# argumentcomputer/lurk-beta

Hardware: AMD Instinct MI355X
Metric: MSM Mscalar-mul/s (Pallas Pedersen commitment, bases+scalars resident in HBM) (higher is better)
Workload: dtype u32x8 (255-bit Montgomery, integer VALU)

## Files before the change

### bench_tools/check_asm_operands.py

```python
#!/usr/bin/env python3
import re
import sys
import os
_CSRC = os.path.join(os.path.dirname(os.path.dirname(os.path.abspath(__file__))), 'lurk_beta_amd', 'csrc')
hdrs = [os.path.join(_CSRC, 'field29_mul_asm.cuh'), os.path.join(_CSRC, 'field_mul_asm.cuh')]
templates = []
for h in hdrs:
    src = open(h).read()
    for m in re.finditer(r'asm(?:\s+volatile)?\(\s*((?:\s*"[^"\n]*"\s*\n?)+)\s*:\s*([^;]*?);', src, re.S):
        lines = [l for l in re.findall(r'"([^"\n]*)"', m.group(1))]
        lines = [l.replace('\\n\\t', '').replace('\\n', '').strip() for l in lines]
        lines = [l for l in lines if l]
        cl = re.findall(r'"([vs]\d+)"', m.group(2).split(':')[-1])
        templates.append((lines, set(cl)))
print("templates:", [(len(t[0]), len(t[1])) for t in templates])
s = open(sys.argv[1]).read()
blocks = re.findall(r';;#ASMSTART\n(.*?);;#ASMEND', s, re.S)
print("asm blocks in .s:", len(blocks))
bad = 0
matched = 0
for b in blocks:
    bl = [l.strip() for l in b.strip().split('\n') if l.strip()]
    cand = [t for t in templates if len(t[0]) == len(bl)]
    if not cand:
        continue
    tl, clob = cand[0]
    for tl, clob in cand:
        ok = True
        ops = {}
        for a, e in zip(tl, bl):
            pat = re.escape(a)
            pat = re.sub(r'%(\d+)', lambda m: r'(?P<o' + m.group(1) + r'>\S+?)', pat.replace('\\%', '%'))
            seen = set()
            def fix(m):
                n = m.group(1)
                if n in seen: return '(?P=o%s)' % n
                seen.add(n); return m.group(0)
            pat = re.sub(r'\(\?P<o(\d+)>\\S\+\?\)', fix, pat)
            mm = re.fullmatch(pat, e)
            if not mm: ok = False; break
            ops.update(mm.groupdict())
        if ok:
            break
    if not ok:
        continue
    matched += 1
    clobnums = {(c[0], int(c[1:])) for c in clob}
    for k, r in ops.items():
        r = r.rstrip(',')
        m1 = re.fullmatch(r'([vs])(\d+)', r); m2 = re.fullmatch(r'([vs])\[(\d+):(\d+)\]', r)
        regs = []
        if m1: regs = [(m1.group(1), int(m1.group(2)))]
        elif m2: regs = [(m2.group(1), i) for i in range(int(m2.group(2)), int(m2.group(3)) + 1)]
        if any(x in clobnums for x in regs):
            bad += 1
            print("OVERLAP: operand %s -> %s is a clobbered scratch register" % (k, r))
print("matched blocks:", matched, "overlaps:", bad)
sys.exit(1 if bad or not matched else 0)
```

### lurk_beta_amd/csrc/curve29.cuh

```cuda
#pragma once
#include "curve.cuh"
#include "field29.cuh"

#ifndef LURK_ACC_Y3_ROW
#define LURK_ACC_Y3_ROW 1
#endif
#ifndef LURK_ACC_AFFINE_FIRST
#define LURK_ACC_AFFINE_FIRST 1
#endif
#ifndef LURK_F29_RARE_ATTR
#define LURK_F29_RARE_ATTR __attribute__((noinline))
#endif

namespace lurk {

template <class P>
LURK_HD F29<P> f29_carry_signed(const int32_t* t) {
    F29<P> r;
    int32_t c = 0;
#pragma unroll
    for (int i = 0; i < 8; i++) {
        int32_t x = t[i] + c;
        r.l[i] = (uint32_t)x & F29_MASK;
        c = x >> 29;
    }
    r.l[8] = (uint32_t)(t[8] + c);
    return r;
}

template <class P>
LURK_HD constexpr bool f29_pasta_shape() {
    return P::NBITS == 255 && f29_mod<P>(0) == 1u && f29_mod<P>(5) == 0u && f29_mod<P>(6) == 0u && f29_mod<P>(7) == 0u;
}

template <class P>
LURK_HD F29<P> f29_reduce_pasta(const F29<P>& v) {
    const uint32_t k = v.l[8] >> 22;
    const uint32_t km1 = k ? k - 1 : 0;
    int32_t t[9];
    uint64_t c = 0;
#pragma unroll
    for (int i = 0; i < 5; i++) {
        c += (uint64_t)km1 * f29_mod<P>(i);
        t[i] = (int32_t)v.l[i] - (int32_t)((uint32_t)c & F29_MASK);
        c >>= 29;
    }
    t[5] = (int32_t)v.l[5] - (int32_t)(uint32_t)c;
    t[6] = (int32_t)v.l[6];
    t[7] = (int32_t)v.l[7];
    t[8] = (int32_t)(v.l[8] & ((1u << 22) - 1u)) + (k ? (int32_t)(1u << 22) : 0);
    return f29_carry_signed<P>(t);
}
template <class P>
LURK_HD F29<P> f29_reduce_general(const F29<P>& v) {
    constexpr uint32_t D = (P::mod(7) >> 8) + 1u;
    static_assert(D > (1u << 21) && D <= (1u << 22), "f29_reduce_general: the modulus must have 253 or 254 bits");
    constexpr uint64_t mu = ((uint64_t)1 << 53) / D;
    F29_ASSERT(v.l[8] < (1u << 31), "f29_reduce: top limb >= 2^31");
    const uint32_t q = (uint32_t)(((uint64_t)v.l[8] * mu) >> 53);
    int32_t t[9];
    uint64_t c = 0;
#pragma unroll
    for (int i = 0; i < 8; i++) {
        c += (uint64_t)q * f29_mod<P>(i);
        t[i] = (int32_t)v.l[i] - (int32_t)((uint32_t)c & F29_MASK);
        c >>= 29;
    }
    c += (uint64_t)q * f29_mod<P>(8);
    t[8] = (int32_t)v.l[8] - (int32_t)(uint32_t)c;
    const F29<P> r = f29_carry_signed<P>(t);
    F29_ASSERT(r.l[8] < (1u << 24), "f29_reduce: result not below 2^256");
    return r;
}
template <class P>
LURK_HD F29<P> f29_reduce(const F29<P>& v) {
    if constexpr (f29_pasta_shape<P>()) return f29_reduce_pasta<P>(v);
    else return f29_reduce_general<P>(v);
}

template <class P>
struct Xyzz29 {
    F29<P> x, y, zz, zzz;
};

template <class P>
LURK_HD Xyzz<P> xyzz29_to_xyzz(const Xyzz29<P>& a, bool is_identity) {
    if (is_identity) return xyzz_identity<P>();
    Xyzz<P> r;
    r.x = f29_to_mont256<P>(a.x);
    r.y = f29_to_mont256<P>(a.y);
    r.zz = f29_to_mont256<P>(a.zz);
    r.zzz = f29_to_mont256<P>(a.zzz);
    return r;
}
template <class P>
LURK_HD void xyzz29_from_xyzz(const Xyzz<P>& a, Xyzz29<P>& r, bool& is_identity) {
    is_identity = xyzz_is_identity<P>(a);
    r.x = f29_from_mont256<P>(a.x);
    r.y = f29_from_mont256<P>(a.y);
    r.zz = f29_from_mont256<P>(a.zz);
    r.zzz = f29_from_mont256<P>(a.zzz);
}

template <class P>
LURK_HD uint32_t f29_multiple_candidate(const F29<P>& v) {
    if constexpr (f29_pasta_shape<P>()) return v.l[0];
    else return (v.l[0] * ((0u - f29_inv<P>()) & F29_MASK)) & F29_MASK;
}
template <class P>
LURK_HD bool f29_maybe_multiple_of_p(const F29<P>& v) {
    return f29_multiple_candidate<P>(v) < (f29_pasta_shape<P>() ? 128u : 256u);
}
template <class P>
LURK_HD bool f29_is_multiple_of_p(const F29<P>& v) {
    const uint32_t k = f29_multiple_candidate<P>(v);
    uint64_t c = 0;
    bool eq = true;
#pragma unroll
    for (int i = 0; i < 8; i++) {
        c += (uint64_t)k * f29_mod<P>(i);
        eq = eq && (v.l[i] == ((uint32_t)c & F29_MASK));
        c >>= 29;
    }
    c += (uint64_t)k * f29_mod<P>(8);
    return eq && (uint64_t)v.l[8] == c;
}

template <class P>
LURK_HD LURK_F29_RARE_ATTR Xyzz29<P> xyzz29_double_affine(F29<P> qx, F29<P> qy_signed) {
    const F29<P> u = f29_dbl<P>(qy_signed);
    const F29<P> v = f29_mul<P>(u, u);
    const F29<P> w = f29_mul<P>(u, v);
    const F29<P> s = f29_mul<P>(qx, v);
    const F29<P> xx = f29_sqr<P>(qx);
    const F29<P> m = f29_carry<P>(f29_add<P>(f29_dbl<P>(xx), xx));
    const F29<P> m2 = f29_sqr<P>(m);
    Xyzz29<P> r;
    r.x = f29_reduce<P>(f29_carry<P>(f29_sub<P>(m2, f29_dbl<P>(s))));
    const F29<P> t1 = f29_mul<P>(m, f29_sub<P>(s, r.x));
    const F29<P> t2 = f29_mul<P>(w, qy_signed);
    r.y = f29_reduce<P>(f29_carry<P>(f29_sub<P>(t1, t2)));
    r.zz = v;
    r.zzz = w;
    return r;
}

template <class P, bool ACC_AFFINE = false>
LURK_HD void xyzz29_madd(Xyzz29<P>& acc, bool& acc_id, const Affine<P>& q, bool negate) {
    if (affine_is_identity<P>(q)) return;
    const F29<P> qx = f29_from_mont256<P>(q.x);
    const F29<P> qy = f29_from_mont256<P>(q.y);
    if (acc_id) {
        acc.x = qx;
        acc.y = negate ? f29_reduce<P>(f29_carry<P>(f29_sub<P>(f29_zero<P>(), qy))) : qy;
        Fe<P> one = fe_one<P>();
        acc.zz = f29_from_mont256<P>(one);
        acc.zzz = acc.zz;
        acc_id = false;
        return;
    }
    F29_ASSERT_LIMBS(acc.x, 29, "acc.x"); F29_ASSERT_TOP(acc.x, 27, "acc.x");
    F29_ASSERT_LIMBS(acc.y, 29, "acc.y"); F29_ASSERT_TOP(acc.y, 27, "acc.y");
    F29_ASSERT_LIMBS(acc.zz, 29, "acc.zz"); F29_ASSERT_TOP(acc.zz, 27, "acc.zz");
    F29_ASSERT_LIMBS(acc.zzz, 29, "acc.zzz"); F29_ASSERT_TOP(acc.zzz, 27, "acc.zzz");
    const F29<P> u2 = ACC_AFFINE ? qx : f29_mul<P>(qx, acc.zz);
    const F29<P> s2 = ACC_AFFINE ? qy : f29_mul<P>(qy, acc.zzz);
    const F29<P> p = f29_carry<P>(f29_sub<P>(u2, acc.x));
    F29<P> r;
#pragma unroll
    for (int i = 0; i < 9; i++) {
        F29_ASSERT(f29_bias<P>(i) >= acc.y.l[i], "madd: Y1 limb above the bias");
        r.l[i] = s2.l[i] + (negate ? acc.y.l[i] : f29_bias<P>(i) - acc.y.l[i]);
    }
    r = f29_carry<P>(r);
    if (f29_maybe_multiple_of_p<P>(p) && f29_is_multiple_of_p<P>(p)) {
        if (f29_maybe_multiple_of_p<P>(r) && f29_is_multiple_of_p<P>(r)) {
            const F29<P> qys = negate ? f29_reduce<P>(f29_carry<P>(f29_sub<P>(f29_zero<P>(), qy))) : qy;
            acc = xyzz29_double_affine<P>(qx, qys);
        } else {
            acc_id = true;
        }
        return;
    }
    const F29<P> pp = f29_sqr<P>(p);
    const F29<P> ppp = f29_mul<P>(p, pp);
    const F29<P> qq = f29_mul<P>(acc.x, pp);
    const F29<P> r2 = f29_sqr<P>(r);
    F29<P> x3 = f29_sub<P>(f29_sub<P>(r2, ppp), f29_dbl<P>(qq));
    x3 = f29_reduce<P>(f29_carry<P>(x3));
    F29<P> d;
#pragma unroll
    for (int i = 0; i < 9; i++) {
        F29_ASSERT(f29_bias<P>(i) >= qq.l[i] && f29_bias<P>(i) >= x3.l[i], "madd: Q / X3 limb above the bias");
        d.l[i] = negate ? x3.l[i] + (f29_bias<P>(i) - qq.l[i]) : qq.l[i] + (f29_bias<P>(i) - x3.l[i]);
    }
#if LURK_ACC_Y3_ROW
    Dot29<P> row;
    dot29_init<P>(row);
    dot29_mac<P>(row, r, f29_carry<P>(d));
    dot29_mac<P>(row, f29_carry<P>(f29_sub<P>(f29_zero<P>(), acc.y)), ppp);
    F29<P> y3 = f29_reduce<P>(dot29_finish<P>(row));
#else
    const F29<P> t1 = f29_mul<P>(r, d);
    const F29<P> t2 = f29_mul<P>(acc.y, ppp);
    F29<P> y3 = f29_reduce<P>(f29_carry<P>(f29_sub<P>(t1, t2)));
#endif
    acc.x = x3;
    acc.y = y3;
    if (ACC_AFFINE) {
        acc.zz = f29_reduce<P>(pp);
        acc.zzz = f29_reduce<P>(ppp);
    } else {
        acc.zz = f29_mul<P>(acc.zz, pp);
        acc.zzz = f29_mul<P>(acc.zzz, ppp);
    }
}

template <class P>
LURK_HD Xyzz29<P> xyzz29_dbl(const Xyzz29<P>& a) {
    const F29<P> u = f29_dbl<P>(a.y);
    const F29<P> v = f29_mul<P>(u, u);
    const F29<P> w = f29_mul<P>(u, v);
    const F29<P> s = f29_mul<P>(a.x, v);
    const F29<P> xx = f29_sqr<P>(a.x);
    const F29<P> m = f29_carry<P>(f29_add<P>(f29_dbl<P>(xx), xx));
    const F29<P> m2 = f29_sqr<P>(m);
    Xyzz29<P> r;
    r.x = f29_reduce<P>(f29_carry<P>(f29_sub<P>(m2, f29_dbl<P>(s))));
    const F29<P> t1 = f29_mul<P>(m, f29_sub<P>(s, r.x));
    const F29<P> t2 = f29_mul<P>(w, a.y);
    r.y = f29_reduce<P>(f29_carry<P>(f29_sub<P>(t1, t2)));
    r.zz = f29_mul<P>(v, a.zz);
    r.zzz = f29_mul<P>(w, a.zzz);
    return r;
}

template <class P>
LURK_HD LURK_F29_RARE_ATTR Xyzz29<P> xyzz29_double_general(Xyzz29<P> a) {
    const Xyzz<P> d = xyzz_dbl<P>(xyzz29_to_xyzz<P>(a, false));
    Xyzz29<P> r;
    bool id;
    xyzz29_from_xyzz<P>(d, r, id);
    return r;
}

template <class P>
LURK_HD void xyzz29_add(Xyzz29<P>& acc, bool& acc_id, const Xyzz29<P>& q, bool q_id) {
    if (q_id) return;
    if (acc_id) {
        acc = q;
        acc_id = false;
        return;
    }
    F29_ASSERT_LIMBS(acc.x, 29, "add acc.x"); F29_ASSERT_TOP(acc.x, 27, "add acc.x");
    F29_ASSERT_LIMBS(acc.y, 29, "add acc.y"); F29_ASSERT_TOP(acc.y, 27, "add acc.y");
    F29_ASSERT_LIMBS(acc.zz, 29, "add acc.zz"); F29_ASSERT_TOP(acc.zz, 27, "add acc.zz");
    F29_ASSERT_LIMBS(acc.zzz, 29, "add acc.zzz"); F29_ASSERT_TOP(acc.zzz, 27, "add acc.zzz");
    F29_ASSERT_LIMBS(q.x, 29, "add q.x"); F29_ASSERT_TOP(q.x, 27, "add q.x");
    F29_ASSERT_LIMBS(q.y, 29, "add q.y"); F29_ASSERT_TOP(q.y, 27, "add q.y");
    F29_ASSERT_LIMBS(q.zz, 29, "add q.zz"); F29_ASSERT_TOP(q.zz, 27, "add q.zz");
    F29_ASSERT_LIMBS(q.zzz, 29, "add q.zzz"); F29_ASSERT_TOP(q.zzz, 27, "add q.zzz");
    const F29<P> u1 = f29_mul<P>(acc.x, q.zz);
    const F29<P> u2 = f29_mul<P>(q.x, acc.zz);
    const F29<P> s1 = f29_mul<P>(acc.y, q.zzz);
    const F29<P> s2 = f29_mul<P>(q.y, acc.zzz);
    const F29<P> p = f29_carry<P>(f29_sub<P>(u2, u1));
    const F29<P> r = f29_carry<P>(f29_sub<P>(s2, s1));
    if (f29_maybe_multiple_of_p<P>(p) && f29_is_multiple_of_p<P>(p)) {
        if (f29_maybe_multiple_of_p<P>(r) && f29_is_multiple_of_p<P>(r)) acc = xyzz29_double_general<P>(acc);
        else acc_id = true;
        return;
    }
    const F29<P> pp = f29_sqr<P>(p);
    const F29<P> ppp = f29_mul<P>(p, pp);
    const F29<P> qq = f29_mul<P>(u1, pp);
    const F29<P> r2 = f29_sqr<P>(r);
    F29<P> x3 = f29_sub<P>(f29_sub<P>(r2, ppp), f29_dbl<P>(qq));
    x3 = f29_reduce<P>(f29_carry<P>(x3));
    F29<P> d;
#pragma unroll
    for (int i = 0; i < 9; i++) {
        F29_ASSERT(f29_bias<P>(i) >= x3.l[i], "add: X3 limb above the bias");
        d.l[i] = qq.l[i] + (f29_bias<P>(i) - x3.l[i]);
    }
    Dot29<P> row;
    dot29_init<P>(row);
    dot29_mac<P>(row, r, f29_carry<P>(d));
    dot29_mac<P>(row, f29_carry<P>(f29_sub<P>(f29_zero<P>(), s1)), ppp);
    const F29<P> y3 = f29_reduce<P>(dot29_finish<P>(row));
    const F29<P> zz12 = f29_mul<P>(acc.zz, q.zz);
    const F29<P> zzz12 = f29_mul<P>(acc.zzz, q.zzz);
    acc.x = x3;
    acc.y = y3;
    acc.zz = f29_mul<P>(zz12, pp);
    acc.zzz = f29_mul<P>(zzz12, ppp);
}

template <class P>
LURK_HD Xyzz<P> xyzz_sum_via29(const Xyzz<P>* pts, uint32_t nt) {
    if (nt == 0) return xyzz_identity<P>();
    if (nt == 1) return pts[0];
    Xyzz29<P> acc, q;
    bool acc_id, q_id;
    xyzz29_from_xyzz<P>(pts[0], acc, acc_id);
    for (uint32_t i = 1; i < nt; i++) {
        xyzz29_from_xyzz<P>(pts[i], q, q_id);
        xyzz29_add<P>(acc, acc_id, q, q_id);
    }
    return xyzz29_to_xyzz<P>(acc, acc_id);
}

template <class P>
LURK_HD void msm_task_accumulate29_raw(const uint32_t* sorted, uint32_t first, uint32_t last, const Affine<P>* table, Xyzz29<P>& acc, bool& acc_id) {
    acc.x = acc.y = acc.zz = acc.zzz = f29_zero<P>();
    acc_id = true;
#if LURK_ACC_AFFINE_FIRST
    uint32_t j = first;
    if (j < last) {
        const uint32_t e = sorted[j++];
        xyzz29_madd<P>(acc, acc_id, table[e & 0x7fffffffu], (e & 0x80000000u) != 0);
    }
    if (j < last) {
        const uint32_t e = sorted[j++];
        const Affine<P> q = table[e & 0x7fffffffu];
#if LURK_ACC_AFFINE_FIRST
        if (!acc_id) xyzz29_madd<P, true>(acc, acc_id, q, (e & 0x80000000u) != 0);
        else
#endif
            xyzz29_madd<P>(acc, acc_id, q, (e & 0x80000000u) != 0);
    }
    for (; j < last; j++) {
        const uint32_t e = sorted[j];
        const Affine<P> q = table[e & 0x7fffffffu];
        xyzz29_madd<P>(acc, acc_id, q, (e & 0x80000000u) != 0);
    }
#else
    for (uint32_t j = first; j < last; j++) {
        const uint32_t e = sorted[j];
#ifdef LURK_ACC_DEBUG_TABLE_MASK
        const Affine<P> q = table[e & LURK_ACC_DEBUG_TABLE_MASK];
#else
        const Affine<P> q = table[e & 0x7fffffffu];
#endif
        xyzz29_madd<P>(acc, acc_id, q, (e & 0x80000000u) != 0);
    }
#endif
}
template <class P>
LURK_HD Xyzz<P> msm_task_accumulate29(const uint32_t* sorted, uint32_t first, uint32_t last, const Affine<P>* table) {
    Xyzz29<P> acc;
    bool acc_id;
    msm_task_accumulate29_raw<P>(sorted, first, last, table, acc, acc_id);
    return xyzz29_to_xyzz<P>(acc, acc_id);
}

}
```

### lurk_beta_amd/csrc/field29.cuh

```cuda
#pragma once
#include "field.cuh"

#if defined(LURK_F29_CHECK) && !defined(__HIP_DEVICE_COMPILE__)
#include <cstdio>
#include <cstdlib>
#define F29_CHECKS_ACTIVE 1
#define F29_ASSERT_LIMBS(v, bits, what)                                                        \
    do {                                                                                       \
        for (int _i = 0; _i < 9; _i++)                                                         \
            if ((uint64_t)(v).l[_i] >> (bits)) { printf("F29 bound violated: %s limb %d = %u (>= 2^%d)\n", what, _i, (v).l[_i], bits); abort(); } \
    } while (0)
#define F29_ASSERT(cond, what)                                                                 \
    do {                                                                                       \
        if (!(cond)) { printf("F29 bound violated: %s\n", what); abort(); }                     \
    } while (0)
#define F29_ASSERT_TOP(v, bits, what)                                                          \
    do {                                                                                       \
        if ((uint64_t)(v).l[8] >> (bits)) { printf("F29 bound violated: %s top limb = %u (>= 2^%d)\n", what, (v).l[8], bits); abort(); } \
    } while (0)
#else
#define F29_ASSERT_LIMBS(v, bits, what) ((void)0)
#define F29_ASSERT_TOP(v, bits, what) ((void)0)
#define F29_ASSERT(cond, what) ((void)0)
#define F29_CHECKS_ACTIVE 0
#endif


namespace lurk {

template <class P>
struct F29 {
    uint32_t l[9];
};

constexpr uint32_t F29_MASK = (1u << 29) - 1u;

template <class P>
LURK_HD constexpr uint32_t f29_mod(int i) {
    const int bit = 29 * i, limb = bit >> 5, sh = bit & 31;
    uint64_t v = limb < 8 ? P::mod(limb) : 0u;
    if (limb + 1 < 8) v |= (uint64_t)P::mod(limb + 1) << 32;
    return (uint32_t)(v >> sh) & F29_MASK;
}
template <class P>
LURK_HD constexpr uint32_t f29_inv() {
    return P::INV & F29_MASK;
}

template <class P>
LURK_HD F29<P> f29_zero() {
    F29<P> z;
#pragma unroll
    for (int i = 0; i < 9; i++) z.l[i] = 0;
    return z;
}

template <class P>
LURK_HD F29<P> f29_carry(const F29<P>& a) {
    F29<P> r;
    uint32_t c = 0;
#pragma unroll
    for (int i = 0; i < 8; i++) {
        uint32_t x = a.l[i] + c;
        r.l[i] = x & F29_MASK;
        c = x >> 29;
    }
    r.l[8] = a.l[8] + c;
    return r;
}

template <class P>
LURK_HD F29<P> f29_add(const F29<P>& a, const F29<P>& b) {
    F29<P> r;
#pragma unroll
    for (int i = 0; i < 9; i++) r.l[i] = a.l[i] + b.l[i];
    return r;
}
template <class P>
LURK_HD constexpr uint32_t f29_bias(int i) {
    uint64_t carry = 0;
    uint32_t limb = 0;
    for (int k = 0; k <= i; k++) {
        uint64_t x = (uint64_t)f29_mod<P>(k) * 64u + carry;
        limb = (uint32_t)(x & F29_MASK);
        carry = x >> 29;
        if (k == 8) limb = (uint32_t)x;
    }
    uint32_t v = limb;
    if (i < 8) v += 1u << 30;
    if (i > 0) v -= 2u;
    return v;
}
template <class P>
LURK_HD F29<P> f29_sub(const F29<P>& a, const F29<P>& b) {
    F29<P> r;
#pragma unroll
    for (int i = 0; i < 9; i++) {
        F29_ASSERT(f29_bias<P>(i) >= b.l[i], "f29_sub: subtrahend limb above the bias (value >= 64p or limbs not tight)");
        r.l[i] = a.l[i] + (f29_bias<P>(i) - b.l[i]);
    }
    return r;
}
template <class P>
LURK_HD F29<P> f29_dbl(const F29<P>& a) {
    F29<P> r;
#pragma unroll
    for (int i = 0; i < 9; i++) r.l[i] = a.l[i] << 1;
    return r;
}

template <class P>
LURK_HD F29<P> f29_mul_portable(const F29<P>& a, const F29<P>& b) {
    uint32_t m[9];
    F29<P> t;
    uint64_t acc = 0;
#if defined(LURK_F29_CHECK) && !defined(__HIP_DEVICE_COMPILE__)
    {
        uint64_t ma = 0, mb = 0;
        for (int i = 0; i < 9; i++) { ma = a.l[i] > ma ? a.l[i] : ma; mb = b.l[i] > mb ? b.l[i] : mb; }
        F29_ASSERT((unsigned __int128)ma * mb * 9 + ((unsigned __int128)10 << 58) < ((unsigned __int128)1 << 64), "f29_mul column overflow");
    }
#endif
#pragma unroll
    for (int k = 0; k < 17; k++) {
#pragma unroll
        for (int i = (k > 8 ? k - 8 : 0); i <= (k < 8 ? k : 8); i++) acc += (uint64_t)a.l[i] * b.l[k - i];
#pragma unroll
        for (int i = (k > 8 ? k - 8 : 0); i <= (k - 1 < 8 ? k - 1 : 8); i++) acc += (uint64_t)m[i] * f29_mod<P>(k - i);
        if (k <= 8) {
            m[k] = ((uint32_t)acc * f29_inv<P>()) & F29_MASK;
            acc += (uint64_t)m[k] * f29_mod<P>(0);
        } else {
            t.l[k - 9] = (uint32_t)acc & F29_MASK;
        }
        acc >>= 29;
    }
    t.l[8] = (uint32_t)acc;
    return t;
}

}
#include "field29_mul_asm.cuh"
#include "field29_mul_asm_bn254fq.cuh"
namespace lurk {

template <class P>
LURK_HD F29<P> f29_mul(const F29<P>& a, const F29<P>& b) {
#if defined(__HIP_DEVICE_COMPILE__)
    return f29_mul_asm<P>(a, b);
#else
    return f29_mul_portable<P>(a, b);
#endif
}
template <class P>
LURK_HD F29<P> f29_sqr(const F29<P>& a) {
#if defined(__HIP_DEVICE_COMPILE__)
    return f29_sqr_asm<P>(a);
#else
    return f29_mul_portable<P>(a, a);
#endif
}

template <class P>
LURK_HD F29<P> f29_invert(const F29<P>& a) {
    uint32_t e[8];
    uint32_t borrow = 2;
    for (int i = 0; i < 8; i++) {
        const uint64_t x = (uint64_t)P::mod(i) - borrow;
        e[i] = (uint32_t)x;
        borrow = (uint32_t)(x >> 63);
    }
    int top = 255;
    while (top > 0 && !((e[top >> 5] >> (top & 31)) & 1u)) top--;
    F29<P> acc = a;
#if defined(__HIP_DEVICE_COMPILE__)
#pragma unroll 1
#endif
    for (int b = top - 1; b >= 0; b--) {
        acc = f29_sqr<P>(acc);
        if ((e[b >> 5] >> (b & 31)) & 1u) acc = f29_mul<P>(acc, a);
    }
    return acc;
}

template <class P>
struct Dot29 {
    uint64_t c[17];
#if defined(LURK_F29_CHECK) && !defined(__HIP_DEVICE_COMPILE__)
    unsigned __int128 shadow[17];
#endif
};
template <class P>
LURK_HD void dot29_init(Dot29<P>& A) {
#pragma unroll
    for (int k = 0; k < 17; k++) A.c[k] = 0;
#if defined(LURK_F29_CHECK) && !defined(__HIP_DEVICE_COMPILE__)
    for (int k = 0; k < 17; k++) A.shadow[k] = 0;
#endif
}
template <class P>
LURK_HD void dot29_mac(Dot29<P>& A, const F29<P>& a, const F29<P>& b) {
#pragma unroll
    for (int i = 0; i < 9; i++)
#pragma unroll
        for (int j = 0; j < 9; j++) A.c[i + j] += (uint64_t)a.l[i] * b.l[j];
#if defined(LURK_F29_CHECK) && !defined(__HIP_DEVICE_COMPILE__)
    for (int i = 0; i < 9; i++)
        for (int j = 0; j < 9; j++) A.shadow[i + j] += (unsigned __int128)a.l[i] * b.l[j];
    for (int k = 0; k < 17; k++) F29_ASSERT(A.shadow[k] + ((unsigned __int128)10 << 58) < ((unsigned __int128)1 << 64), "dot29 column overflow");
#endif
}
template <class P>
LURK_HD void dot29_carry(Dot29<P>& A) {
#pragma unroll
    for (int k = 0; k < 16; k++) {
        A.c[k + 1] += A.c[k] >> 29;
        A.c[k] &= F29_MASK;
    }
#if defined(LURK_F29_CHECK) && !defined(__HIP_DEVICE_COMPILE__)
    for (int k = 0; k < 17; k++) A.shadow[k] = A.c[k];
#endif
}
template <class P>
LURK_HD F29<P> dot29_finish(const Dot29<P>& A) {
    uint32_t m[9];
    F29<P> t;
    uint64_t acc = 0;
#pragma unroll
    for (int k = 0; k < 17; k++) {
        acc += A.c[k];
#pragma unroll
        for (int i = (k > 8 ? k - 8 : 0); i <= (k - 1 < 8 ? k - 1 : 8); i++) acc += (uint64_t)m[i] * f29_mod<P>(k - i);
        if (k <= 8) {
            m[k] = ((uint32_t)acc * f29_inv<P>()) & F29_MASK;
            acc += (uint64_t)m[k] * f29_mod<P>(0);
        } else {
            t.l[k - 9] = (uint32_t)acc & F29_MASK;
        }
        acc >>= 29;
    }
    t.l[8] = (uint32_t)acc;
    return t;
}

template <class P>
LURK_HD F29<P> f29_from_mont256(const Fe<P>& x) {
    F29<P> r;
#pragma unroll
    for (int i = 0; i < 9; i++) {
        const int bit = 29 * i - 5;
        uint64_t v;
        if (bit < 0) {
            v = (uint64_t)x.l[0] << 5;
        } else {
            const int limb = bit >> 5, sh = bit & 31;
            v = limb < 8 ? x.l[limb] : 0u;
            if (limb + 1 < 8) v |= (uint64_t)x.l[limb + 1] << 32;
            v >>= sh;
        }
        r.l[i] = (uint32_t)v & F29_MASK;
    }
    return r;
}
template <class P>
LURK_HD F29<P> f29_from_plain(const uint32_t* x) {
    F29<P> r;
#pragma unroll
    for (int i = 0; i < 9; i++) {
        const int bit = 29 * i, limb = bit >> 5, sh = bit & 31;
        uint64_t v = limb < 8 ? x[limb] : 0u;
        if (limb + 1 < 8) v |= (uint64_t)x[limb + 1] << 32;
        r.l[i] = (uint32_t)(v >> sh) & F29_MASK;
    }
    return r;
}
template <class P>
LURK_HD void f29_pack(const F29<P>& a, uint32_t* out) {
#pragma unroll
    for (int w = 0; w < 8; w++) {
        const int bit = 32 * w, i = bit / 29, sh = bit % 29;
        uint64_t v = (uint64_t)a.l[i] >> sh;
        if (i + 1 < 9) v |= (uint64_t)a.l[i + 1] << (29 - sh);
        if (i + 2 < 9) v |= (uint64_t)a.l[i + 2] << (58 - sh);
        out[w] = (uint32_t)v;
    }
}
template <class P>
LURK_HD F29<P> f29_const_r256() {
    uint32_t r[8];
#pragma unroll
    for (int i = 0; i < 8; i++) r[i] = P::r(i);
    return f29_from_plain<P>(r);
}
template <class P>
LURK_HD Fe<P> f29_to_mont256(const F29<P>& a) {
    F29<P> u = f29_mul<P>(f29_carry<P>(a), f29_const_r256<P>());
    uint32_t w[8];
    f29_pack<P>(u, w);
    fe_cond_sub2<P>(w);
    fe_cond_sub<P>(w);
    Fe<P> r;
#pragma unroll
    for (int i = 0; i < 8; i++) r.l[i] = w[i];
    return r;
}

}
```

### lurk_beta_amd/csrc/gen_field29_asm.py

```python
#!/usr/bin/env python3
import sys

FIELDS = {
    "PallasFp": 0x40000000000000000000000000000000224698FC094CF91B992D30ED00000001,
    "PallasFq": 0x40000000000000000000000000000000224698FC0994A8DD8C46EB2100000001,
    "Bn254Fr": 0x30644E72E131A029B85045B68181585D2833E84879B9709143E1F593F0000001,
}
BN254FQ_FIELDS = {
    "Bn254Fq": 0x30644E72E131A029B85045B68181585D97816A916871CA8D3C208C16D87CFD47,
}
W = 29
MASK = (1 << W) - 1
ACC_LO, ACC_HI = 16, 17
M_BASE = 18
P_SGPR_BASE = 4
INV_SGPR = 13
MASK_VGPR = 27
DUMMY = 16
P_VGPR_BASE = 28
MOD_IN_VGPR = False
LAST_VGPR = P_VGPR_BASE + 8 if MOD_IN_VGPR else MASK_VGPR


def limbs29(x):
    return [(x >> (W * i)) & MASK for i in range(9)]


def gen_mul(modulus, square=False):
    p = limbs29(modulus)
    inv = (-pow(modulus, -1, 1 << W)) % (1 << W)
    L = []
    T = lambda i: f"%{i}"
    A = lambda i: f"%{9 + i}"
    B = lambda i: f"%{18 + i}"
    M = lambda i: f"v{M_BASE + i}"

    def P(j):
        if p[j] == 1:
            return "1"
        return f"v{P_VGPR_BASE + j}" if MOD_IN_VGPR else f"s{P_SGPR_BASE + j}"

    for j in range(9):
        if p[j] not in (0, 1):
            if MOD_IN_VGPR:
                L.append(f"v_mov_b32 v{P_VGPR_BASE + j}, 0x{p[j]:08x}")
            else:
                L.append(f"s_mov_b32 s{P_SGPR_BASE + j}, 0x{p[j]:08x}")
    if inv != MASK:
        L.append(f"s_mov_b32 s{INV_SGPR}, 0x{inv:08x}")
    L.append(f"v_mov_b32 v{MASK_VGPR}, 0x{MASK:08x}")
    first = True
    for k in range(17):
        if square:
            prods = [(A(i), B(k - i)) for i in range(max(0, k - 8), min(k, 8) + 1) if i < k - i]
            if k % 2 == 0:
                prods.append((A(k // 2), A(k // 2)))
        else:
            prods = [(A(i), B(k - i)) for i in range(max(0, k - 8), min(k, 8) + 1)]
        prods += [(M(i), P(k - i)) for i in range(max(0, k - 8), min(k - 1, 8) + 1) if p[k - i] != 0]
        for x, y in prods:
            src2 = "0" if first else f"v[{ACC_LO}:{ACC_HI}]"
            L.append(f"v_mad_u64_u32 v[{ACC_LO}:{ACC_HI}], s[{DUMMY}:{DUMMY + 1}], {x}, {y}, {src2}")
            first = False
        if k <= 8:
            if inv == MASK:
                L.append(f"v_sub_u32 {M(k)}, 0, v{ACC_LO}")
            else:
                L.append(f"v_mul_lo_u32 {M(k)}, v{ACC_LO}, s{INV_SGPR}")
            L.append(f"v_and_b32 {M(k)}, v{MASK_VGPR}, {M(k)}")
            L.append(f"v_mad_u64_u32 v[{ACC_LO}:{ACC_HI}], s[{DUMMY}:{DUMMY + 1}], {M(k)}, {P(0)}, v[{ACC_LO}:{ACC_HI}]")
        else:
            L.append(f"v_and_b32 {T(k - 9)}, v{MASK_VGPR}, v{ACC_LO}")
        if k < 16:
            L.append(f"v_lshrrev_b64 v[{ACC_LO}:{ACC_HI}], {W}, v[{ACC_LO}:{ACC_HI}]")
    L.append(f"v_lshrrev_b64 v[{ACC_LO}:{ACC_HI}], {W}, v[{ACC_LO}:{ACC_HI}]")
    L.append(f"v_mov_b32 {T(8)}, v{ACC_LO}")
    return L, p, inv


def cxx_sqr(name, modulus):
    lines, p, inv = gen_mul(modulus, square=True)
    nmad = sum(1 for l in lines if l.startswith("v_mad"))
    body = "\n".join(f'        "{l}\\n\\t"' for l in lines)
    outs = ", ".join(f'"=&v"(t.l[{i}])' for i in range(9))
    ins = ", ".join([f'"v"(a.l[{i}])' for i in range(9)] + [f'"v"(d.l[{i}])' for i in range(9)])
    vclob = ", ".join(f'"v{r}"' for r in range(ACC_LO, LAST_VGPR + 1))
    sclob = ", ".join(f'"s{r}"' for r in range(P_SGPR_BASE, DUMMY + 2))
    return f"""// {name} squaring: {nmad} v_mad_u64_u32 (cross products once, against the doubled operand)
template <>
__device__ __forceinline__ F29<{name}> f29_sqr_asm<{name}>(const F29<{name}>& a) {{
    F29<{name}> t, d;
#pragma unroll
    for (int i = 0; i < 9; i++) d.l[i] = a.l[i] << 1;
    asm(
{body}
        : {outs}
        : {ins}
        : {vclob}, {sclob}, "vcc");
    return t;
}}
"""


def cxx(name, modulus):
    lines, p, inv = gen_mul(modulus)
    nmad = sum(1 for l in lines if l.startswith("v_mad"))
    nvalu = sum(1 for l in lines if l.startswith("v_"))
    body = "\n".join(f'        "{l}\\n\\t"' for l in lines)
    outs = ", ".join(f'"=&v"(t.l[{i}])' for i in range(9))
    ins = ", ".join([f'"v"(a.l[{i}])' for i in range(9)] + [f'"v"(b.l[{i}])' for i in range(9)])
    vclob = ", ".join(f'"v{r}"' for r in range(ACC_LO, LAST_VGPR + 1))
    sclob = ", ".join(f'"s{r}"' for r in range(P_SGPR_BASE, DUMMY + 2))
    return f"""// {name}: {nmad} v_mad_u64_u32, {nvalu} VALU instructions, no carry folds
template <>
__device__ __forceinline__ F29<{name}> f29_mul_asm<{name}>(const F29<{name}>& a, const F29<{name}>& b) {{
    F29<{name}> t;
    asm(
{body}
        : {outs}
        : {ins}
        : {vclob}, {sclob}, "vcc");
    return t;
}}
"""


def main():
    bn254fq = sys.argv[1:] == ["--bn254fq"]
    out = [
        "// field29_mul_asm_bn254fq.cuh - GENERATED by gen_field29_asm.py --bn254fq; do not edit." if bn254fq else
        "// field29_mul_asm.cuh - GENERATED by gen_field29_asm.py; do not edit.",
        "#pragma once",
        "#if defined(__HIP_DEVICE_COMPILE__)",
        "namespace lurk {",
    ]
    if not bn254fq:
        out += [
            "template <class P> __device__ __forceinline__ F29<P> f29_mul_asm(const F29<P>& a, const F29<P>& b);",
            "template <class P> __device__ __forceinline__ F29<P> f29_sqr_asm(const F29<P>& a);",
        ]
    out.append("")
    for name, mod in (BN254FQ_FIELDS if bn254fq else FIELDS).items():
        out.append(cxx(name, mod))
        out.append(cxx_sqr(name, mod))
    out += ["}  // namespace lurk", "#endif"]
    sys.stdout.write("\n".join(out) + "\n")


if __name__ == "__main__":
    main()
```

Measured before the change: 1020.

## Add p≡1 mod 2^29 Montgomery variant using signed carry for Pasta field muls

Adds a second Montgomery multiply/square path for Pasta fields, whose modulus is 1 mod 2^29. It derives the per-column quotient with a bitwise NOT of a biased accumulator instead of a negate, and carries with an arithmetic shift. Most multiplications in the XYZZ add, double and madd formulas, plus the Y3 dot-row finish, now call this path through new mul30/sqr30 wrappers. The aim is to shorten the VALU instruction chain per field multiply, at the cost of tighter column-overflow bounds that now depend on operand limb sizes.

Result: faster. 1058 (median of 6 runs) (+3.8%).

```diff
diff --git a/bench_tools/check_asm_operands.py b/bench_tools/check_asm_operands.py
--- a/bench_tools/check_asm_operands.py
+++ b/bench_tools/check_asm_operands.py
@@ -3,7 +3,7 @@
 import sys
 import os
 _CSRC = os.path.join(os.path.dirname(os.path.dirname(os.path.abspath(__file__))), 'lurk_beta_amd', 'csrc')
-hdrs = [os.path.join(_CSRC, 'field29_mul_asm.cuh'), os.path.join(_CSRC, 'field_mul_asm.cuh')]
+hdrs = [os.path.join(_CSRC, 'field29_mul_asm.cuh'), os.path.join(_CSRC, 'field29_mul_asm_p1.cuh'), os.path.join(_CSRC, 'field_mul_asm.cuh')]
 templates = []
 for h in hdrs:
     src = open(h).read()
diff --git a/lurk_beta_amd/csrc/curve29.cuh b/lurk_beta_amd/csrc/curve29.cuh
--- a/lurk_beta_amd/csrc/curve29.cuh
+++ b/lurk_beta_amd/csrc/curve29.cuh
@@ -28,10 +28,6 @@
     return r;
 }
 
-template <class P>
-LURK_HD constexpr bool f29_pasta_shape() {
-    return P::NBITS == 255 && f29_mod<P>(0) == 1u && f29_mod<P>(5) == 0u && f29_mod<P>(6) == 0u && f29_mod<P>(7) == 0u;
-}
 
 template <class P>
 LURK_HD F29<P> f29_reduce_pasta(const F29<P>& v) {
@@ -130,15 +126,15 @@
 LURK_HD LURK_F29_RARE_ATTR Xyzz29<P> xyzz29_double_affine(F29<P> qx, F29<P> qy_signed) {
     const F29<P> u = f29_dbl<P>(qy_signed);
     const F29<P> v = f29_mul<P>(u, u);
-    const F29<P> w = f29_mul<P>(u, v);
-    const F29<P> s = f29_mul<P>(qx, v);
-    const F29<P> xx = f29_sqr<P>(qx);
+    const F29<P> w = f29_mul30<P>(u, v);
+    const F29<P> s = f29_mul30<P>(qx, v);
+    const F29<P> xx = f29_sqr30<P>(qx);
     const F29<P> m = f29_carry<P>(f29_add<P>(f29_dbl<P>(xx), xx));
-    const F29<P> m2 = f29_sqr<P>(m);
+    const F29<P> m2 = f29_sqr30<P>(m);
     Xyzz29<P> r;
     r.x = f29_reduce<P>(f29_carry<P>(f29_sub<P>(m2, f29_dbl<P>(s))));
     const F29<P> t1 = f29_mul<P>(m, f29_sub<P>(s, r.x));
-    const F29<P> t2 = f29_mul<P>(w, qy_signed);
+    const F29<P> t2 = f29_mul30<P>(w, qy_signed);
     r.y = f29_reduce<P>(f29_carry<P>(f29_sub<P>(t1, t2)));
     r.zz = v;
     r.zzz = w;
@@ -163,8 +159,8 @@
     F29_ASSERT_LIMBS(acc.y, 29, "acc.y"); F29_ASSERT_TOP(acc.y, 27, "acc.y");
     F29_ASSERT_LIMBS(acc.zz, 29, "acc.zz"); F29_ASSERT_TOP(acc.zz, 27, "acc.zz");
     F29_ASSERT_LIMBS(acc.zzz, 29, "acc.zzz"); F29_ASSERT_TOP(acc.zzz, 27, "acc.zzz");
-    const F29<P> u2 = ACC_AFFINE ? qx : f29_mul<P>(qx, acc.zz);
-    const F29<P> s2 = ACC_AFFINE ? qy : f29_mul<P>(qy, acc.zzz);
+    const F29<P> u2 = ACC_AFFINE ? qx : f29_mul30<P>(qx, acc.zz);
+    const F29<P> s2 = ACC_AFFINE ? qy : f29_mul30<P>(qy, acc.zzz);
     const F29<P> p = f29_carry<P>(f29_sub<P>(u2, acc.x));
     F29<P> r;
 #pragma unroll
@@ -182,10 +178,10 @@
         }
         return;
     }
-    const F29<P> pp = f29_sqr<P>(p);
-    const F29<P> ppp = f29_mul<P>(p, pp);
-    const F29<P> qq = f29_mul<P>(acc.x, pp);
-    const F29<P> r2 = f29_sqr<P>(r);
+    const F29<P> pp = f29_sqr30<P>(p);
+    const F29<P> ppp = f29_mul30<P>(p, pp);
+    const F29<P> qq = f29_mul30<P>(acc.x, pp);
+    const F29<P> r2 = f29_sqr30<P>(r);
     F29<P> x3 = f29_sub<P>(f29_sub<P>(r2, ppp), f29_dbl<P>(qq));
     x3 = f29_reduce<P>(f29_carry<P>(x3));
     F29<P> d;
@@ -199,10 +195,10 @@
     dot29_init<P>(row);
     dot29_mac<P>(row, r, f29_carry<P>(d));
     dot29_mac<P>(row, f29_carry<P>(f29_sub<P>(f29_zero<P>(), acc.y)), ppp);
-    F29<P> y3 = f29_reduce<P>(dot29_finish<P>(row));
+    F29<P> y3 = f29_reduce<P>(dot29_finish2<P>(row));
 #else
     const F29<P> t1 = f29_mul<P>(r, d);
-    const F29<P> t2 = f29_mul<P>(acc.y, ppp);
+    const F29<P> t2 = f29_mul30<P>(acc.y, ppp);
     F29<P> y3 = f29_reduce<P>(f29_carry<P>(f29_sub<P>(t1, t2)));
 #endif
     acc.x = x3;
@@ -211,8 +207,8 @@
         acc.zz = f29_reduce<P>(pp);
         acc.zzz = f29_reduce<P>(ppp);
     } else {
-        acc.zz = f29_mul<P>(acc.zz, pp);
-        acc.zzz = f29_mul<P>(acc.zzz, ppp);
+        acc.zz = f29_mul30<P>(acc.zz, pp);
+        acc.zzz = f29_mul30<P>(acc.zzz, ppp);
     }
 }
 
@@ -220,18 +216,18 @@
 LURK_HD Xyzz29<P> xyzz29_dbl(const Xyzz29<P>& a) {
     const F29<P> u = f29_dbl<P>(a.y);
     const F29<P> v = f29_mul<P>(u, u);
-    const F29<P> w = f29_mul<P>(u, v);
-    const F29<P> s = f29_mul<P>(a.x, v);
-    const F29<P> xx = f29_sqr<P>(a.x);
+    const F29<P> w = f29_mul30<P>(u, v);
+    const F29<P> s = f29_mul30<P>(a.x, v);
+    const F29<P> xx = f29_sqr30<P>(a.x);
     const F29<P> m = f29_carry<P>(f29_add<P>(f29_dbl<P>(xx), xx));
-    const F29<P> m2 = f29_sqr<P>(m);
+    const F29<P> m2 = f29_sqr30<P>(m);
     Xyzz29<P> r;
     r.x = f29_reduce<P>(f29_carry<P>(f29_sub<P>(m2, f29_dbl<P>(s))));
     const F29<P> t1 = f29_mul<P>(m, f29_sub<P>(s, r.x));
-    const F29<P> t2 = f29_mul<P>(w, a.y);
+    const F29<P> t2 = f29_mul30<P>(w, a.y);
     r.y = f29_reduce<P>(f29_carry<P>(f29_sub<P>(t1, t2)));
-    r.zz = f29_mul<P>(v, a.zz);
-    r.zzz = f29_mul<P>(w, a.zzz);
+    r.zz = f29_mul30<P>(v, a.zz);
+    r.zzz = f29_mul30<P>(w, a.zzz);
     return r;
 }
 
@@ -260,10 +256,10 @@
     F29_ASSERT_LIMBS(q.y, 29, "add q.y"); F29_ASSERT_TOP(q.y, 27, "add q.y");
     F29_ASSERT_LIMBS(q.zz, 29, "add q.zz"); F29_ASSERT_TOP(q.zz, 27, "add q.zz");
     F29_ASSERT_LIMBS(q.zzz, 29, "add q.zzz"); F29_ASSERT_TOP(q.zzz, 27, "add q.zzz");
-    const F29<P> u1 = f29_mul<P>(acc.x, q.zz);
-    const F29<P> u2 = f29_mul<P>(q.x, acc.zz);
-    const F29<P> s1 = f29_mul<P>(acc.y, q.zzz);
-    const F29<P> s2 = f29_mul<P>(q.y, acc.zzz);
+    const F29<P> u1 = f29_mul30<P>(acc.x, q.zz);
+    const F29<P> u2 = f29_mul30<P>(q.x, acc.zz);
+    const F29<P> s1 = f29_mul30<P>(acc.y, q.zzz);
+    const F29<P> s2 = f29_mul30<P>(q.y, acc.zzz);
     const F29<P> p = f29_carry<P>(f29_sub<P>(u2, u1));
     const F29<P> r = f29_carry<P>(f29_sub<P>(s2, s1));
     if (f29_maybe_multiple_of_p<P>(p) && f29_is_multiple_of_p<P>(p)) {
@@ -271,10 +267,10 @@
         else acc_id = true;
         return;
     }
-    const F29<P> pp = f29_sqr<P>(p);
-    const F29<P> ppp = f29_mul<P>(p, pp);
-    const F29<P> qq = f29_mul<P>(u1, pp);
-    const F29<P> r2 = f29_sqr<P>(r);
+    const F29<P> pp = f29_sqr30<P>(p);
+    const F29<P> ppp = f29_mul30<P>(p, pp);
+    const F29<P> qq = f29_mul30<P>(u1, pp);
+    const F29<P> r2 = f29_sqr30<P>(r);
     F29<P> x3 = f29_sub<P>(f29_sub<P>(r2, ppp), f29_dbl<P>(qq));
     x3 = f29_reduce<P>(f29_carry<P>(x3));
     F29<P> d;
@@ -287,13 +283,13 @@
     dot29_init<P>(row);
     dot29_mac<P>(row, r, f29_carry<P>(d));
     dot29_mac<P>(row, f29_carry<P>(f29_sub<P>(f29_zero<P>(), s1)), ppp);
-    const F29<P> y3 = f29_reduce<P>(dot29_finish<P>(row));
-    const F29<P> zz12 = f29_mul<P>(acc.zz, q.zz);
-    const F29<P> zzz12 = f29_mul<P>(acc.zzz, q.zzz);
+    const F29<P> y3 = f29_reduce<P>(dot29_finish2<P>(row));
+    const F29<P> zz12 = f29_mul30<P>(acc.zz, q.zz);
+    const F29<P> zzz12 = f29_mul30<P>(acc.zzz, q.zzz);
     acc.x = x3;
     acc.y = y3;
-    acc.zz = f29_mul<P>(zz12, pp);
-    acc.zzz = f29_mul<P>(zzz12, ppp);
+    acc.zz = f29_mul30<P>(zz12, pp);
+    acc.zzz = f29_mul30<P>(zzz12, ppp);
 }
 
 template <class P>
diff --git a/lurk_beta_amd/csrc/field29.cuh b/lurk_beta_amd/csrc/field29.cuh
--- a/lurk_beta_amd/csrc/field29.cuh
+++ b/lurk_beta_amd/csrc/field29.cuh
@@ -1,5 +1,9 @@
 #pragma once
 #include "field.cuh"
+
+#ifndef LURK_F29_P1
+#define LURK_F29_P1 1
+#endif
 
 #if defined(LURK_F29_CHECK) && !defined(__HIP_DEVICE_COMPILE__)
 #include <cstdio>
@@ -48,6 +52,15 @@
 }
 
 template <class P>
+LURK_HD constexpr bool f29_pasta_shape() {
+    return P::NBITS == 255 && f29_mod<P>(0) == 1u && f29_mod<P>(5) == 0u && f29_mod<P>(6) == 0u && f29_mod<P>(7) == 0u;
+}
+template <class P>
+LURK_HD constexpr bool f29_p1_form() {
+    return LURK_F29_P1 != 0 && f29_pasta_shape<P>() && f29_inv<P>() == F29_MASK;
+}
+
+template <class P>
 LURK_HD F29<P> f29_zero() {
     F29<P> z;
 #pragma unroll
@@ -139,9 +152,46 @@
     return t;
 }
 
+template <class P>
+LURK_HD F29<P> f29_mul30_portable(const F29<P>& a, const F29<P>& b) {
+    if constexpr (!f29_p1_form<P>()) {
+        return f29_mul_portable<P>(a, b);
+    } else {
+        uint32_t m[9];
+        F29<P> t;
+        uint64_t acc = ~(uint64_t)0;
+#if defined(LURK_F29_CHECK) && !defined(__HIP_DEVICE_COMPILE__)
+        {
+            uint64_t ma = 0, mb = 0;
+            for (int i = 0; i < 9; i++) { ma = a.l[i] > ma ? a.l[i] : ma; mb = b.l[i] > mb ? b.l[i] : mb; }
+            F29_ASSERT((unsigned __int128)ma * mb * 9 + ((unsigned __int128)5 << 58) + ((unsigned __int128)1 << 36) < ((unsigned __int128)1 << 63), "f29_mul column overflow");
+        }
+#endif
+#pragma unroll
+        for (int k = 0; k < 17; k++) {
+#pragma unroll
+            for (int i = (k > 8 ? k - 8 : 0); i <= (k < 8 ? k : 8); i++) acc += (uint64_t)a.l[i] * b.l[k - i];
+#pragma unroll
+            for (int i = (k > 8 ? k - 8 : 0); i <= (k - 1 < 8 ? k - 1 : 8); i++) acc += (uint64_t)m[i] * f29_mod<P>(k - i);
+            if (k <= 8) {
+                F29_ASSERT((int64_t)acc >= -1, "f29_mul column overflow");
+                m[k] = ~(uint32_t)acc & F29_MASK;
+                acc = (uint64_t)((int64_t)acc >> 29);
+                if (k == 8) acc += 1;
+            } else {
+                t.l[k - 9] = (uint32_t)acc & F29_MASK;
+                acc >>= 29;
+            }
+        }
+        t.l[8] = (uint32_t)acc;
+        return t;
+    }
+}
+
 }
 #include "field29_mul_asm.cuh"
 #include "field29_mul_asm_bn254fq.cuh"
+#include "field29_mul_asm_p1.cuh"
 namespace lurk {
 
 template <class P>
@@ -153,11 +203,29 @@
 #endif
 }
 template <class P>
+LURK_HD F29<P> f29_mul30(const F29<P>& a, const F29<P>& b) {
+#if defined(__HIP_DEVICE_COMPILE__)
+    if constexpr (f29_p1_form<P>()) return f29_mul_p1_asm<P>(a, b);
+    else return f29_mul_asm<P>(a, b);
+#else
+    return f29_mul30_portable<P>(a, b);
+#endif
+}
+template <class P>
 LURK_HD F29<P> f29_sqr(const F29<P>& a) {
 #if defined(__HIP_DEVICE_COMPILE__)
     return f29_sqr_asm<P>(a);
 #else
     return f29_mul_portable<P>(a, a);
+#endif
+}
+template <class P>
+LURK_HD F29<P> f29_sqr30(const F29<P>& a) {
+#if defined(__HIP_DEVICE_COMPILE__)
+    if constexpr (f29_p1_form<P>()) return f29_sqr_p1_asm<P>(a);
+    else return f29_sqr_asm<P>(a);
+#else
+    return f29_mul30_portable<P>(a, a);
 #endif
 }
 
@@ -177,8 +245,8 @@
 #pragma unroll 1
 #endif
     for (int b = top - 1; b >= 0; b--) {
-        acc = f29_sqr<P>(acc);
-        if ((e[b >> 5] >> (b & 31)) & 1u) acc = f29_mul<P>(acc, a);
+        acc = f29_sqr30<P>(acc);
+        if ((e[b >> 5] >> (b & 31)) & 1u) acc = f29_mul30<P>(acc, a);
     }
     return acc;
 }
@@ -241,6 +309,38 @@
     }
     t.l[8] = (uint32_t)acc;
     return t;
+}
+
+template <class P>
+LURK_HD F29<P> dot29_finish2(const Dot29<P>& A) {
+    if constexpr (!f29_p1_form<P>()) {
+        return dot29_finish<P>(A);
+    } else {
+        uint32_t m[9];
+        F29<P> t;
+        uint64_t acc = ~(uint64_t)0;
+#if defined(LURK_F29_CHECK) && !defined(__HIP_DEVICE_COMPILE__)
+        for (int k = 0; k < 17; k++)
+            F29_ASSERT(A.shadow[k] + ((unsigned __int128)5 << 58) + ((unsigned __int128)1 << 36) < ((unsigned __int128)1 << 63), "dot29 column overflow");
+#endif
+#pragma unroll
+        for (int k = 0; k < 17; k++) {
+            acc += A.c[k];
+#pragma unroll
+            for (int i = (k > 8 ? k - 8 : 0); i <= (k - 1 < 8 ? k - 1 : 8); i++) acc += (uint64_t)m[i] * f29_mod<P>(k - i);
+            if (k <= 8) {
+                F29_ASSERT((int64_t)acc >= -1, "dot29 column overflow");
+                m[k] = ~(uint32_t)acc & F29_MASK;
+                acc = (uint64_t)((int64_t)acc >> 29);
+                if (k == 8) acc += 1;
+            } else {
+                t.l[k - 9] = (uint32_t)acc & F29_MASK;
+                acc >>= 29;
+            }
+        }
+        t.l[8] = (uint32_t)acc;
+        return t;
+    }
 }
 
 template <class P>
@@ -294,7 +394,7 @@
 }
 template <class P>
 LURK_HD Fe<P> f29_to_mont256(const F29<P>& a) {
-    F29<P> u = f29_mul<P>(f29_carry<P>(a), f29_const_r256<P>());
+    F29<P> u = f29_mul30<P>(f29_carry<P>(a), f29_const_r256<P>());
     uint32_t w[8];
     f29_pack<P>(u, w);
     fe_cond_sub2<P>(w);
diff --git a/lurk_beta_amd/csrc/field29_mul_asm_p1.cuh b/lurk_beta_amd/csrc/field29_mul_asm_p1.cuh
--- /dev/null
+++ b/lurk_beta_amd/csrc/field29_mul_asm_p1.cuh
@@ -0,0 +1,688 @@
+#pragma once
+#if defined(__HIP_DEVICE_COMPILE__)
+namespace lurk {
+template <class P> __device__ __forceinline__ F29<P> f29_mul_p1_asm(const F29<P>& a, const F29<P>& b);
+template <class P> __device__ __forceinline__ F29<P> f29_sqr_p1_asm(const F29<P>& a);
+
+template <>
+__device__ __forceinline__ F29<PallasFp> f29_mul_p1_asm<PallasFp>(const F29<PallasFp>& a, const F29<PallasFp>& b) {
+    F29<PallasFp> t;
+    asm(
+        "s_mov_b32 s5, 0x09698768\n\t"
+        "s_mov_b32 s6, 0x133e46e6\n\t"
+        "s_mov_b32 s7, 0x0d31f812\n\t"
+        "s_mov_b32 s8, 0x00000224\n\t"
+        "s_mov_b32 s12, 0x00400000\n\t"
+        "v_mov_b32 v27, 0x1fffffff\n\t"
+        "v_mad_u64_u32 v[16:17], s[16:17], %9, %18, -1\n\t"
+        "v_not_b32 v18, v16\n\t"
+        "v_and_b32 v18, v27, v18\n\t"
+        "v_ashrrev_i64 v[16:17], 29, v[16:17]\n\t"
+        "v_mad_u64_u32 v[16:17], s[16:17], %9, %19, v[16:17]\n\t"
+        "v_mad_u64_u32 v[16:17], s[16:17], %10, %18, v[16:17]\n\t"
+        "v_mad_u64_u32 v[16:17], s[16:17], v18, s5, v[16:17]\n\t"
+        "v_not_b32 v19, v16\n\t"
+        "v_and_b32 v19, v27, v19\n\t"
+        "v_ashrrev_i64 v[16:17], 29, v[16:17]\n\t"
+        "v_mad_u64_u32 v[16:17], s[16:17], %9, %20, v[16:17]\n\t"
+        "v_mad_u64_u32 v[16:17], s[16:17], %10, %19, v[16:17]\n\t"
+        "v_mad_u64_u32 v[16:17], s[16:17], %11, %18, v[16:17]\n\t"
+        "v_mad_u64_u32 v[16:17], s[16:17], v18, s6, v[16:17]\n\t"
+        "v_mad_u64_u32 v[16:17], s[16:17], v19, s5, v[16:17]\n\t"
+        "v_not_b32 v20, v16\n\t"
+        "v_and_b32 v20, v27, v20\n\t"
+        "v_ashrrev_i64 v[16:17], 29, v[16:17]\n\t"
+        "v_mad_u64_u32 v[16:17], s[16:17], %9, %21, v[16:17]\n\t"
+        "v_mad_u64_u32 v[16:17], s[16:17], %10, %20, v[16:17]\n\t"
+        "v_mad_u64_u32 v[16:17], s[16:17], %11, %19, v[16:17]\n\t"
+        "v_mad_u64_u32 v[16:17], s[16:17], %12, %18, v[16:17]\n\t"
+        "v_mad_u64_u32 v[16:17], s[16:17], v18, s7, v[16:17]\n\t"
+        "v_mad_u64_u32 v[16:17], s[16:17], v19, s6, v[16:17]\n\t"
+        "v_mad_u64_u32 v[16:17], s[16:17], v20, s5, v[16:17]\n\t"
+        "v_not_b32 v21, v16\n\t"
+        "v_and_b32 v21, v27, v21\n\t"
+        "v_ashrrev_i64 v[16:17], 29, v[16:17]\n\t"
+        "v_mad_u64_u32 v[16:17], s[16:17], %9, %22, v[16:17]\n\t"
+        "v_mad_u64_u32 v[16:17], s[16:17], %10, %21, v[16:17]\n\t"
+        "v_mad_u64_u32 v[16:17], s[16:17], %11, %20, v[16:17]\n\t"
+        "v_mad_u64_u32 v[16:17], s[16:17], %12, %19, v[16:17]\n\t"
+        "v_mad_u64_u32 v[16:17], s[16:17], %13, %18, v[16:17]\n\t"
+        "v_mad_u64_u32 v[16:17], s[16:17], v18, s8, v[16:17]\n\t"
+        "v_mad_u64_u32 v[16:17], s[16:17], v19, s7, v[16:17]\n\t"
+        "v_mad_u64_u32 v[16:17], s[16:17], v20, s6, v[16:17]\n\t"
+        "v_mad_u64_u32 v[16:17], s[16:17], v21, s5, v[16:17]\n\t"
+        "v_not_b32 v22, v16\n\t"
+        "v_and_b32 v22, v27, v22\n\t"
+        "v_ashrrev_i64 v[16:17], 29, v[16:17]\n\t"
+        "v_mad_u64_u32 v[16:17], s[16:17], %9, %23, v[16:17]\n\t"
+        "v_mad_u64_u32 v[16:17], s[16:17], %10, %22, v[16:17]\n\t"
+        "v_mad_u64_u32 v[16:17], s[16:17], %11, %21, v[16:17]\n\t"
+        "v_mad_u64_u32 v[16:17], s[16:17], %12, %20, v[16:17]\n\t"
+        "v_mad_u64_u32 v[16:17], s[16:17], %13, %19, v[16:17]\n\t"
+        "v_mad_u64_u32 v[16:17], s[16:17], %14, %18, v[16:17]\n\t"
+        "v_mad_u64_u32 v[16:17], s[16:17], v19, s8, v[16:17]\n\t"
+        "v_mad_u64_u32 v[16:17], s[16:17], v20, s7, v[16:17]\n\t"
+        "v_mad_u64_u32 v[16:17], s[16:17], v21, s6, v[16:17]\n\t"
+        "v_mad_u64_u32 v[16:17], s[16:17], v22, s5, v[16:17]\n\t"
+        "v_not_b32 v23, v16\n\t"
+        "v_and_b32 v23, v27, v23\n\t"
+        "v_ashrrev_i64 v[16:17], 29, v[16:17]\n\t"
+        "v_mad_u64_u32 v[16:17], s[16:17], %9, %24, v[16:17]\n\t"
+        "v_mad_u64_u32 v[16:17], s[16:17], %10, %23, v[16:17]\n\t"
+        "v_mad_u64_u32 v[16:17], s[16:17], %11, %22, v[16:17]\n\t"
+        "v_mad_u64_u32 v[16:17], s[16:17], %12, %21, v[16:17]\n\t"
+        "v_mad_u64_u32 v[16:17], s[16:17], %13, %20, v[16:17]\n\t"
+        "v_mad_u64_u32 v[16:17], s[16:17], %14, %19, v[16:17]\n\t"
+        "v_mad_u64_u32 v[16:17], s[16:17], %15, %18, v[16:17]\n\t"
+        "v_mad_u64_u32 v[16:17], s[16:17], v20, s8, v[16:17]\n\t"
+        "v_mad_u64_u32 v[16:17], s[16:17], v21, s7, v[16:17]\n\t"
+        "v_mad_u64_u32 v[16:17], s[16:17], v22, s6, v[16:17]\n\t"
+        "v_mad_u64_u32 v[16:17], s[16:17], v23, s5, v[16:17]\n\t"
+        "v_not_b32 v24, v16\n\t"
+        "v_and_b32 v24, v27, v24\n\t"
+        "v_ashrrev_i64 v[16:17], 29, v[16:17]\n\t"
+        "v_mad_u64_u32 v[16:17], s[16:17], %9, %25, v[16:17]\n\t"
+        "v_mad_u64_u32 v[16:17], s[16:17], %10, %24, v[16:17]\n\t"
+        "v_mad_u64_u32 v[16:17], s[16:17], %11, %23, v[16:17]\n\t"
+        "v_mad_u64_u32 v[16:17], s[16:17], %12, %22, v[16:17]\n\t"
+        "v_mad_u64_u32 v[16:17], s[16:17], %13, %21, v[16:17]\n\t"
+        "v_mad_u64_u32 v[16:17], s[16:17], %14, %20, v[16:17]\n\t"
+        "v_mad_u64_u32 v[16:17], s[16:17], %15, %19, v[16:17]\n\t"
+        "v_mad_u64_u32 v[16:17], s[16:17], %16, %18, v[16:17]\n\t"
+        "v_mad_u64_u32 v[16:17], s[16:17], v21, s8, v[16:17]\n\t"
+        "v_mad_u64_u32 v[16:17], s[16:17], v22, s7, v[16:17]\n\t"
+        "v_mad_u64_u32 v[16:17], s[16:17], v23, s6, v[16:17]\n\t"
+        "v_mad_u64_u32 v[16:17], s[16:17], v24, s5, v[16:17]\n\t"
+        "v_not_b32 v25, v16\n\t"
+        "v_and_b32 v25, v27, v25\n\t"
+        "v_ashrrev_i64 v[16:17], 29, v[16:17]\n\t"
+        "v_mad_u64_u32 v[16:17], s[16:17], %9, %26, v[16:17]\n\t"
+        "v_mad_u64_u32 v[16:17], s[16:17], %10, %25, v[16:17]\n\t"
+        "v_mad_u64_u32 v[16:17], s[16:17], %11, %24, v[16:17]\n\t"
+        "v_mad_u64_u32 v[16:17], s[16:17], %12, %23, v[16:17]\n\t"
+        "v_mad_u64_u32 v[16:17], s[16:17], %13, %22, v[16:17]\n\t"
+        "v_mad_u64_u32 v[16:17], s[16:17], %14, %21, v[16:17]\n\t"
+        "v_mad_u64_u32 v[16:17], s[16:17], %15, %20, v[16:17]\n\t"
+        "v_mad_u64_u32 v[16:17], s[16:17], %16, %19, v[16:17]\n\t"
+        "v_mad_u64_u32 v[16:17], s[16:17], %17, %18, v[16:17]\n\t"
+        "v_mad_u64_u32 v[16:17], s[16:17], v18, s12, v[16:17]\n\t"
+        "v_mad_u64_u32 v[16:17], s[16:17], v22, s8, v[16:17]\n\t"
+        "v_mad_u64_u32 v[16:17], s[16:17], v23, s7, v[16:17]\n\t"
+        "v_mad_u64_u32 v[16:17], s[16:17], v24, s6, v[16:17]\n\t"
+        "v_mad_u64_u32 v[16:17], s[16:17], v25, s5, v[16:17]\n\t"
+        "v_not_b32 v26, v16\n\t"
+        "v_and_b32 v26, v27, v26\n\t"
+        "v_ashrrev_i64 v[16:17], 29, v[16:17]\n\t"
+        "v_lshl_add_u64 v[16:17], v[16:17], 0, 1\n\t"
+        "v_mad_u64_u32 v[16:17], s[16:17], %10, %26, v[16:17]\n\t"
+        "v_mad_u64_u32 v[16:17], s[16:17], %11, %25, v[16:17]\n\t"
+        "v_mad_u64_u32 v[16:17], s[16:17], %12, %24, v[16:17]\n\t"
+        "v_mad_u64_u32 v[16:17], s[16:17], %13, %23, v[16:17]\n\t"
+        "v_mad_u64_u32 v[16:17], s[16:17], %14, %22, v[16:17]\n\t"
+        "v_mad_u64_u32 v[16:17], s[16:17], %15, %21, v[16:17]\n\t"
+        "v_mad_u64_u32 v[16:17], s[16:17], %16, %20, v[16:17]\n\t"
+        "v_mad_u64_u32 v[16:17], s[16:17], %17, %19, v[16:17]\n\t"
+        "v_mad_u64_u32 v[16:17], s[16:17], v19, s12, v[16:17]\n\t"
+        "v_mad_u64_u32 v[16:17], s[16:17], v23, s8, v[16:17]\n\t"
+        "v_mad_u64_u32 v[16:17], s[16:17], v24, s7, v[16:17]\n\t"
+        "v_mad_u64_u32 v[16:17], s[16:17], v25, s6, v[16:17]\n\t"
+        "v_mad_u64_u32 v[16:17], s[16:17], v26, s5, v[16:17]\n\t"
+        "v_and_b32 %0, v27, v16\n\t"
+        "v_lshrrev_b64 v[16:17], 29, v[16:17]\n\t"
+        "v_mad_u64_u32 v[16:17], s[16:17], %11, %26, v[16:17]\n\t"
+        "v_mad_u64_u32 v[16:17], s[16:17], %12, %25, v[16:17]\n\t"
+        "v_mad_u64_u32 v[16:17], s[16:17], %13, %24, v[16:17]\n\t"
+        "v_mad_u64_u32 v[16:17], s[16:17], %14, %23, v[16:17]\n\t"
+        "v_mad_u64_u32 v[16:17], s[16:17], %15, %22, v[16:17]\n\t"
+        "v_mad_u64_u32 v[16:17], s[16:17], %16, %21, v[16:17]\n\t"
+        "v_mad_u64_u32 v[16:17], s[16:17], %17, %20, v[16:17]\n\t"
+        "v_mad_u64_u32 v[16:17], s[16:17], v20, s12, v[16:17]\n\t"
+        "v_mad_u64_u32 v[16:17], s[16:17], v24, s8, v[16:17]\n\t"
+        "v_mad_u64_u32 v[16:17], s[16:17], v25, s7, v[16:17]\n\t"
+        "v_mad_u64_u32 v[16:17], s[16:17], v26, s6, v[16:17]\n\t"
+        "v_and_b32 %1, v27, v16\n\t"
+        "v_lshrrev_b64 v[16:17], 29, v[16:17]\n\t"
+        "v_mad_u64_u32 v[16:17], s[16:17], %12, %26, v[16:17]\n\t"
+        "v_mad_u64_u32 v[16:17], s[16:17], %13, %25, v[16:17]\n\t"
+        "v_mad_u64_u32 v[16:17], s[16:17], %14, %24, v[16:17]\n\t"
+        "v_mad_u64_u32 v[16:17], s[16:17], %15, %23, v[16:17]\n\t"
+        "v_mad_u64_u32 v[16:17], s[16:17], %16, %22, v[16:17]\n\t"
+        "v_mad_u64_u32 v[16:17], s[16:17], %17, %21, v[16:17]\n\t"
+        "v_mad_u64_u32 v[16:17], s[16:17], v21, s12, v[16:17]\n\t"
+        "v_mad_u64_u32 v[16:17], s[16:17], v25, s8, v[16:17]\n\t"
+        "v_mad_u64_u32 v[16:17], s[16:17], v26, s7, v[16:17]\n\t"
+        "v_and_b32 %2, v27, v16\n\t"
+        "v_lshrrev_b64 v[16:17], 29, v[16:17]\n\t"
+        "v_mad_u64_u32 v[16:17], s[16:17], %13, %26, v[16:17]\n\t"
+        "v_mad_u64_u32 v[16:17], s[16:17], %14, %25, v[16:17]\n\t"
+        "v_mad_u64_u32 v[16:17], s[16:17], %15, %24, v[16:17]\n\t"
+        "v_mad_u64_u32 v[16:17], s[16:17], %16, %23, v[16:17]\n\t"
+        "v_mad_u64_u32 v[16:17], s[16:17], %17, %22, v[16:17]\n\t"
+        "v_mad_u64_u32 v[16:17], s[16:17], v22, s12, v[16:17]\n\t"
+        "v_mad_u64_u32 v[16:17], s[16:17], v26, s8, v[16:17]\n\t"
+        "v_and_b32 %3, v27, v16\n\t"
+        "v_lshrrev_b64 v[16:17], 29, v[16:17]\n\t"
+        "v_mad_u64_u32 v[16:17], s[16:17], %14, %26, v[16:17]\n\t"
+        "v_mad_u64_u32 v[16:17], s[16:17], %15, %25, v[16:17]\n\t"
+        "v_mad_u64_u32 v[16:17], s[16:17], %16, %24, v[16:17]\n\t"
+        "v_mad_u64_u32 v[16:17], s[16:17], %17, %23, v[16:17]\n\t"
+        "v_mad_u64_u32 v[16:17], s[16:17], v23, s12, v[16:17]\n\t"
+        "v_and_b32 %4, v27, v16\n\t"
+        "v_lshrrev_b64 v[16:17], 29, v[16:17]\n\t"
+        "v_mad_u64_u32 v[16:17], s[16:17], %15, %26, v[16:17]\n\t"
+        "v_mad_u64_u32 v[16:17], s[16:17], %16, %25, v[16:17]\n\t"
+        "v_mad_u64_u32 v[16:17], s[16:17], %17, %24, v[16:17]\n\t"
+        "v_mad_u64_u32 v[16:17], s[16:17], v24, s12, v[16:17]\n\t"
+        "v_and_b32 %5, v27, v16\n\t"
+        "v_lshrrev_b64 v[16:17], 29, v[16:17]\n\t"
+        "v_mad_u64_u32 v[16:17], s[16:17], %16, %26, v[16:17]\n\t"
+        "v_mad_u64_u32 v[16:17], s[16:17], %17, %25, v[16:17]\n\t"
+        "v_mad_u64_u32 v[16:17], s[16:17], v25, s12, v[16:17]\n\t"
+        "v_and_b32 %6, v27, v16\n\t"
+        "v_lshrrev_b64 v[16:17], 29, v[16:17]\n\t"
+        "v_mad_u64_u32 v[16:17], s[16:17], %17, %26, v[16:17]\n\t"
+        "v_mad_u64_u32 v[16:17], s[16:17], v26, s12, v[16:17]\n\t"
+        "v_and_b32 %7, v27, v16\n\t"
+        "v_lshrrev_b64 v[16:17], 29, v[16:17]\n\t"
+        "v_mov_b32 %8, v16\n\t"
+        : "=&v"(t.l[0]), "=&v"(t.l[1]), "=&v"(t.l[2]), "=&v"(t.l[3]), "=&v"(t.l[4]), "=&v"(t.l[5]), "=&v"(t.l[6]), "=&v"(t.l[7]), "=&v"(t.l[8])
+        : "v"(a.l[0]), "v"(a.l[1]), "v"(a.l[2]), "v"(a.l[3]), "v"(a.l[4]), "v"(a.l[5]), "v"(a.l[6]), "v"(a.l[7]), "v"(a.l[8]), "v"(b.l[0]), "v"(b.l[1]), "v"(b.l[2]), "v"(b.l[3]), "v"(b.l[4]), "v"(b.l[5]), "v"(b.l[6]), "v"(b.l[7]), "v"(b.l[8])
+        : "v16", "v17", "v18", "v19", "v20", "v21", "v22", "v23", "v24", "v25", "v26", "v27", "s4", "s5", "s6", "s7", "s8", "s9", "s10", "s11", "s12", "s13", "s14", "s15", "s16", "s17", "vcc");
+    return t;
+}
+
+template <>
+__device__ __forceinline__ F29<PallasFp> f29_sqr_p1_asm<PallasFp>(const F29<PallasFp>& a) {
+    F29<PallasFp> t, d;
+#pragma unroll
+    for (int i = 0; i < 9; i++) d.l[i] = a.l[i] << 1;
+    asm(
+        "s_mov_b32 s5, 0x09698768\n\t"
+        "s_mov_b32 s6, 0x133e46e6\n\t"
+        "s_mov_b32 s7, 0x0d31f812\n\t"
+        "s_mov_b32 s8, 0x00000224\n\t"
+        "s_mov_b32 s12, 0x00400000\n\t"
+        "v_mov_b32 v27, 0x1fffffff\n\t"
+        "v_mad_u64_u32 v[16:17], s[16:17], %9, %9, -1\n\t"
+        "v_not_b32 v18, v16\n\t"
+        "v_and_b32 v18, v27, v18\n\t"
+        "v_ashrrev_i64 v[16:17], 29, v[16:17]\n\t"
+        "v_mad_u64_u32 v[16:17], s[16:17], %9, %19, v[16:17]\n\t"
+        "v_mad_u64_u32 v[16:17], s[16:17], v18, s5, v[16:17]\n\t"
+        "v_not_b32 v19, v16\n\t"
+        "v_and_b32 v19, v27, v19\n\t"
+        "v_ashrrev_i64 v[16:17], 29, v[16:17]\n\t"
+        "v_mad_u64_u32 v[16:17], s[16:17], %9, %20, v[16:17]\n\t"
+        "v_mad_u64_u32 v[16:17], s[16:17], %10, %10, v[16:17]\n\t"
+        "v_mad_u64_u32 v[16:17], s[16:17], v18, s6, v[16:17]\n\t"
+        "v_mad_u64_u32 v[16:17], s[16:17], v19, s5, v[16:17]\n\t"
+        "v_not_b32 v20, v16\n\t"
+        "v_and_b32 v20, v27, v20\n\t"
+        "v_ashrrev_i64 v[16:17], 29, v[16:17]\n\t"
+        "v_mad_u64_u32 v[16:17], s[16:17], %9, %21, v[16:17]\n\t"
+        "v_mad_u64_u32 v[16:17], s[16:17], %10, %20, v[16:17]\n\t"
+        "v_mad_u64_u32 v[16:17], s[16:17], v18, s7, v[16:17]\n\t"
+        "v_mad_u64_u32 v[16:17], s[16:17], v19, s6, v[16:17]\n\t"
+        "v_mad_u64_u32 v[16:17], s[16:17], v20, s5, v[16:17]\n\t"
+        "v_not_b32 v21, v16\n\t"
+        "v_and_b32 v21, v27, v21\n\t"
+        "v_ashrrev_i64 v[16:17], 29, v[16:17]\n\t"
+        "v_mad_u64_u32 v[16:17], s[16:17], %9, %22, v[16:17]\n\t"
+        "v_mad_u64_u32 v[16:17], s[16:17], %10, %21, v[16:17]\n\t"
+        "v_mad_u64_u32 v[16:17], s[16:17], %11, %11, v[16:17]\n\t"
+        "v_mad_u64_u32 v[16:17], s[16:17], v18, s8, v[16:17]\n\t"
+        "v_mad_u64_u32 v[16:17], s[16:17], v19, s7, v[16:17]\n\t"
+        "v_mad_u64_u32 v[16:17], s[16:17], v20, s6, v[16:17]\n\t"
+        "v_mad_u64_u32 v[16:17], s[16:17], v21, s5, v[16:17]\n\t"
+        "v_not_b32 v22, v16\n\t"
+        "v_and_b32 v22, v27, v22\n\t"
+        "v_ashrrev_i64 v[16:17], 29, v[16:17]\n\t"
+        "v_mad_u64_u32 v[16:17], s[16:17], %9, %23, v[16:17]\n\t"
+        "v_mad_u64_u32 v[16:17], s[16:17], %10, %22, v[16:17]\n\t"
+        "v_mad_u64_u32 v[16:17], s[16:17], %11, %21, v[16:17]\n\t"
+        "v_mad_u64_u32 v[16:17], s[16:17], v19, s8, v[16:17]\n\t"
+        "v_mad_u64_u32 v[16:17], s[16:17], v20, s7, v[16:17]\n\t"
+        "v_mad_u64_u32 v[16:17], s[16:17], v21, s6, v[16:17]\n\t"
+        "v_mad_u64_u32 v[16:17], s[16:17], v22, s5, v[16:17]\n\t"
+        "v_not_b32 v23, v16\n\t"
+        "v_and_b32 v23, v27, v23\n\t"
+        "v_ashrrev_i64 v[16:17], 29, v[16:17]\n\t"
+        "v_mad_u64_u32 v[16:17], s[16:17], %9, %24, v[16:17]\n\t"
+        "v_mad_u64_u32 v[16:17], s[16:17], %10, %23, v[16:17]\n\t"
+        "v_mad_u64_u32 v[16:17], s[16:17], %11, %22, v[16:17]\n\t"
+        "v_mad_u64_u32 v[16:17], s[16:17], %12, %12, v[16:17]\n\t"
+        "v_mad_u64_u32 v[16:17], s[16:17], v20, s8, v[16:17]\n\t"
+        "v_mad_u64_u32 v[16:17], s[16:17], v21, s7, v[16:17]\n\t"
+        "v_mad_u64_u32 v[16:17], s[16:17], v22, s6, v[16:17]\n\t"
+        "v_mad_u64_u32 v[16:17], s[16:17], v23, s5, v[16:17]\n\t"
+        "v_not_b32 v24, v16\n\t"
+        "v_and_b32 v24, v27, v24\n\t"
+        "v_ashrrev_i64 v[16:17], 29, v[16:17]\n\t"
+        "v_mad_u64_u32 v[16:17], s[16:17], %9, %25, v[16:17]\n\t"
+        "v_mad_u64_u32 v[16:17], s[16:17], %10, %24, v[16:17]\n\t"
+        "v_mad_u64_u32 v[16:17], s[16:17], %11, %23, v[16:17]\n\t"
+        "v_mad_u64_u32 v[16:17], s[16:17], %12, %22, v[16:17]\n\t"
+        "v_mad_u64_u32 v[16:17], s[16:17], v21, s8, v[16:17]\n\t"
+        "v_mad_u64_u32 v[16:17], s[16:17], v22, s7, v[16:17]\n\t"
+        "v_mad_u64_u32 v[16:17], s[16:17], v23, s6, v[16:17]\n\t"
+        "v_mad_u64_u32 v[16:17], s[16:17], v24, s5, v[16:17]\n\t"
+        "v_not_b32 v25, v16\n\t"
+        "v_and_b32 v25, v27, v25\n\t"
+        "v_ashrrev_i64 v[16:17], 29, v[16:17]\n\t"
+        "v_mad_u64_u32 v[16:17], s[16:17], %9, %26, v[16:17]\n\t"
+        "v_mad_u64_u32 v[16:17], s[16:17], %10, %25, v[16:17]\n\t"
+        "v_mad_u64_u32 v[16:17], s[16:17], %11, %24, v[16:17]\n\t"
+        "v_mad_u64_u32 v[16:17], s[16:17], %12, %23, v[16:17]\n\t"
+        "v_mad_u64_u32 v[16:17], s[16:17], %13, %13, v[16:17]\n\t"
+        "v_mad_u64_u32 v[16:17], s[16:17], v18, s12, v[16:17]\n\t"
+        "v_mad_u64_u32 v[16:17], s[16:17], v22, s8, v[16:17]\n\t"
+        "v_mad_u64_u32 v[16:17], s[16:17], v23, s7, v[16:17]\n\t"
+        "v_mad_u64_u32 v[16:17], s[16:17], v24, s6, v[16:17]\n\t"
+        "v_mad_u64_u32 v[16:17], s[16:17], v25, s5, v[16:17]\n\t"
+        "v_not_b32 v26, v16\n\t"
+        "v_and_b32 v26, v27, v26\n\t"
+        "v_ashrrev_i64 v[16:17], 29, v[16:17]\n\t"
+        "v_lshl_add_u64 v[16:17], v[16:17], 0, 1\n\t"
+        "v_mad_u64_u32 v[16:17], s[16:17], %10, %26, v[16:17]\n\t"
+        "v_mad_u64_u32 v[16:17], s[16:17], %11, %25, v[16:17]\n\t"
+        "v_mad_u64_u32 v[16:17], s[16:17], %12, %24, v[16:17]\n\t"
+        "v_mad_u64_u32 v[16:17], s[16:17], %13, %23, v[16:17]\n\t"
+        "v_mad_u64_u32 v[16:17], s[16:17], v19, s12, v[16:17]\n\t"
+        "v_mad_u64_u32 v[16:17], s[16:17], v23, s8, v[16:17]\n\t"
+        "v_mad_u64_u32 v[16:17], s[16:17], v24, s7, v[16:17]\n\t"
+        "v_mad_u64_u32 v[16:17], s[16:17], v25, s6, v[16:17]\n\t"
+        "v_mad_u64_u32 v[16:17], s[16:17], v26, s5, v[16:17]\n\t"
+        "v_and_b32 %0, v27, v16\n\t"
+        "v_lshrrev_b64 v[16:17], 29, v[16:17]\n\t"
+        "v_mad_u64_u32 v[16:17], s[16:17], %11, %26, v[16:17]\n\t"
+        "v_mad_u64_u32 v[16:17], s[16:17], %12, %25, v[16:17]\n\t"
+        "v_mad_u64_u32 v[16:17], s[16:17], %13, %24, v[16:17]\n\t"
+        "v_mad_u64_u32 v[16:17], s[16:17], %14, %14, v[16:17]\n\t"
+        "v_mad_u64_u32 v[16:17], s[16:17], v20, s12, v[16:17]\n\t"
+        "v_mad_u64_u32 v[16:17], s[16:17], v24, s8, v[16:17]\n\t"
+        "v_mad_u64_u32 v[16:17], s[16:17], v25, s7, v[16:17]\n\t"
+        "v_mad_u64_u32 v[16:17], s[16:17], v26, s6, v[16:17]\n\t"
+        "v_and_b32 %1, v27, v16\n\t"
+        "v_lshrrev_b64 v[16:17], 29, v[16:17]\n\t"
+        "v_mad_u64_u32 v[16:17], s[16:17], %12, %26, v[16:17]\n\t"
+        "v_mad_u64_u32 v[16:17], s[16:17], %13, %25, v[16:17]\n\t"
+        "v_mad_u64_u32 v[16:17], s[16:17], %14, %24, v[16:17]\n\t"
+        "v_mad_u64_u32 v[16:17], s[16:17], v21, s12, v[16:17]\n\t"
+        "v_mad_u64_u32 v[16:17], s[16:17], v25, s8, v[16:17]\n\t"
+        "v_mad_u64_u32 v[16:17], s[16:17], v26, s7, v[16:17]\n\t"
+        "v_and_b32 %2, v27, v16\n\t"
+        "v_lshrrev_b64 v[16:17], 29, v[16:17]\n\t"
+        "v_mad_u64_u32 v[16:17], s[16:17], %13, %26, v[16:17]\n\t"
+        "v_mad_u64_u32 v[16:17], s[16:17], %14, %25, v[16:17]\n\t"
+        "v_mad_u64_u32 v[16:17], s[16:17], %15, %15, v[16:17]\n\t"
+        "v_mad_u64_u32 v[16:17], s[16:17], v22, s12, v[16:17]\n\t"
+        "v_mad_u64_u32 v[16:17], s[16:17], v26, s8, v[16:17]\n\t"
+        "v_and_b32 %3, v27, v16\n\t"
+        "v_lshrrev_b64 v[16:17], 29, v[16:17]\n\t"
+        "v_mad_u64_u32 v[16:17], s[16:17], %14, %26, v[16:17]\n\t"
+        "v_mad_u64_u32 v[16:17], s[16:17], %15, %25, v[16:17]\n\t"
+        "v_mad_u64_u32 v[16:17], s[16:17], v23, s12, v[16:17]\n\t"
+        "v_and_b32 %4, v27, v16\n\t"
+        "v_lshrrev_b64 v[16:17], 29, v[16:17]\n\t"
+        "v_mad_u64_u32 v[16:17], s[16:17], %15, %26, v[16:17]\n\t"
+        "v_mad_u64_u32 v[16:17], s[16:17], %16, %16, v[16:17]\n\t"
+        "v_mad_u64_u32 v[16:17], s[16:17], v24, s12, v[16:17]\n\t"
+        "v_and_b32 %5, v27, v16\n\t"
+        "v_lshrrev_b64 v[16:17], 29, v[16:17]\n\t"
+        "v_mad_u64_u32 v[16:17], s[16:17], %16, %26, v[16:17]\n\t"
+        "v_mad_u64_u32 v[16:17], s[16:17], v25, s12, v[16:17]\n\t"
+        "v_and_b32 %6, v27, v16\n\t"
+        "v_lshrrev_b64 v[16:17], 29, v[16:17]\n\t"
+        "v_mad_u64_u32 v[16:17], s[16:17], %17, %17, v[16:17]\n\t"
+        "v_mad_u64_u32 v[16:17], s[16:17], v26, s12, v[16:17]\n\t"
+        "v_and_b32 %7, v27, v16\n\t"
+        "v_lshrrev_b64 v[16:17], 29, v[16:17]\n\t"
+        "v_mov_b32 %8, v16\n\t"
+        : "=&v"(t.l[0]), "=&v"(t.l[1]), "=&v"(t.l[2]), "=&v"(t.l[3]), "=&v"(t.l[4]), "=&v"(t.l[5]), "=&v"(t.l[6]), "=&v"(t.l[7]), "=&v"(t.l[8])
+        : "v"(a.l[0]), "v"(a.l[1]), "v"(a.l[2]), "v"(a.l[3]), "v"(a.l[4]), "v"(a.l[5]), "v"(a.l[6]), "v"(a.l[7]), "v"(a.l[8]), "v"(d.l[0]), "v"(d.l[1]), "v"(d.l[2]), "v"(d.l[3]), "v"(d.l[4]), "v"(d.l[5]), "v"(d.l[6]), "v"(d.l[7]), "v"(d.l[8])
+        : "v16", "v17", "v18", "v19", "v20", "v21", "v22", "v23", "v24", "v25", "v26", "v27", "s4", "s5", "s6", "s7", "s8", "s9", "s10", "s11", "s12", "s13", "s14", "s15", "s16", "s17", "vcc");
+    return t;
+}
+
+template <>
+__device__ __forceinline__ F29<PallasFq> f29_mul_p1_asm<PallasFq>(const F29<PallasFq>& a, const F29<PallasFq>& b) {
+    F29<PallasFq> t;
+    asm(
+        "s_mov_b32 s5, 0x02375908\n\t"
+        "s_mov_b32 s6, 0x052a3763\n\t"
+        "s_mov_b32 s7, 0x0d31f813\n\t"
+        "s_mov_b32 s8, 0x00000224\n\t"
+        "s_mov_b32 s12, 0x00400000\n\t"
+        "v_mov_b32 v27, 0x1fffffff\n\t"
+        "v_mad_u64_u32 v[16:17], s[16:17], %9, %18, -1\n\t"
+        "v_not_b32 v18, v16\n\t"
+        "v_and_b32 v18, v27, v18\n\t"
+        "v_ashrrev_i64 v[16:17], 29, v[16:17]\n\t"
+        "v_mad_u64_u32 v[16:17], s[16:17], %9, %19, v[16:17]\n\t"
+        "v_mad_u64_u32 v[16:17], s[16:17], %10, %18, v[16:17]\n\t"
+        "v_mad_u64_u32 v[16:17], s[16:17], v18, s5, v[16:17]\n\t"
+        "v_not_b32 v19, v16\n\t"
+        "v_and_b32 v19, v27, v19\n\t"
+        "v_ashrrev_i64 v[16:17], 29, v[16:17]\n\t"
+        "v_mad_u64_u32 v[16:17], s[16:17], %9, %20, v[16:17]\n\t"
+        "v_mad_u64_u32 v[16:17], s[16:17], %10, %19, v[16:17]\n\t"
+        "v_mad_u64_u32 v[16:17], s[16:17], %11, %18, v[16:17]\n\t"
+        "v_mad_u64_u32 v[16:17], s[16:17], v18, s6, v[16:17]\n\t"
+        "v_mad_u64_u32 v[16:17], s[16:17], v19, s5, v[16:17]\n\t"
+        "v_not_b32 v20, v16\n\t"
+        "v_and_b32 v20, v27, v20\n\t"
+        "v_ashrrev_i64 v[16:17], 29, v[16:17]\n\t"
+        "v_mad_u64_u32 v[16:17], s[16:17], %9, %21, v[16:17]\n\t"
+        "v_mad_u64_u32 v[16:17], s[16:17], %10, %20, v[16:17]\n\t"
+        "v_mad_u64_u32 v[16:17], s[16:17], %11, %19, v[16:17]\n\t"
+        "v_mad_u64_u32 v[16:17], s[16:17], %12, %18, v[16:17]\n\t"
+        "v_mad_u64_u32 v[16:17], s[16:17], v18, s7, v[16:17]\n\t"
+        "v_mad_u64_u32 v[16:17], s[16:17], v19, s6, v[16:17]\n\t"
+        "v_mad_u64_u32 v[16:17], s[16:17], v20, s5, v[16:17]\n\t"
+        "v_not_b32 v21, v16\n\t"
+        "v_and_b32 v21, v27, v21\n\t"
+        "v_ashrrev_i64 v[16:17], 29, v[16:17]\n\t"
+        "v_mad_u64_u32 v[16:17], s[16:17], %9, %22, v[16:17]\n\t"
+        "v_mad_u64_u32 v[16:17], s[16:17], %10, %21, v[16:17]\n\t"
+        "v_mad_u64_u32 v[16:17], s[16:17], %11, %20, v[16:17]\n\t"
+        "v_mad_u64_u32 v[16:17], s[16:17], %12, %19, v[16:17]\n\t"
+        "v_mad_u64_u32 v[16:17], s[16:17], %13, %18, v[16:17]\n\t"
+        "v_mad_u64_u32 v[16:17], s[16:17], v18, s8, v[16:17]\n\t"
+        "v_mad_u64_u32 v[16:17], s[16:17], v19, s7, v[16:17]\n\t"
+        "v_mad_u64_u32 v[16:17], s[16:17], v20, s6, v[16:17]\n\t"
+        "v_mad_u64_u32 v[16:17], s[16:17], v21, s5, v[16:17]\n\t"
+        "v_not_b32 v22, v16\n\t"
+        "v_and_b32 v22, v27, v22\n\t"
+        "v_ashrrev_i64 v[16:17], 29, v[16:17]\n\t"
+        "v_mad_u64_u32 v[16:17], s[16:17], %9, %23, v[16:17]\n\t"
+        "v_mad_u64_u32 v[16:17], s[16:17], %10, %22, v[16:17]\n\t"
+        "v_mad_u64_u32 v[16:17], s[16:17], %11, %21, v[16:17]\n\t"
+        "v_mad_u64_u32 v[16:17], s[16:17], %12, %20, v[16:17]\n\t"
+        "v_mad_u64_u32 v[16:17], s[16:17], %13, %19, v[16:17]\n\t"
+        "v_mad_u64_u32 v[16:17], s[16:17], %14, %18, v[16:17]\n\t"
+        "v_mad_u64_u32 v[16:17], s[16:17], v19, s8, v[16:17]\n\t"
+        "v_mad_u64_u32 v[16:17], s[16:17], v20, s7, v[16:17]\n\t"
+        "v_mad_u64_u32 v[16:17], s[16:17], v21, s6, v[16:17]\n\t"
+        "v_mad_u64_u32 v[16:17], s[16:17], v22, s5, v[16:17]\n\t"
+        "v_not_b32 v23, v16\n\t"
+        "v_and_b32 v23, v27, v23\n\t"
+        "v_ashrrev_i64 v[16:17], 29, v[16:17]\n\t"
+        "v_mad_u64_u32 v[16:17], s[16:17], %9, %24, v[16:17]\n\t"
+        "v_mad_u64_u32 v[16:17], s[16:17], %10, %23, v[16:17]\n\t"
+        "v_mad_u64_u32 v[16:17], s[16:17], %11, %22, v[16:17]\n\t"
+        "v_mad_u64_u32 v[16:17], s[16:17], %12, %21, v[16:17]\n\t"
+        "v_mad_u64_u32 v[16:17], s[16:17], %13, %20, v[16:17]\n\t"
+        "v_mad_u64_u32 v[16:17], s[16:17], %14, %19, v[16:17]\n\t"
+        "v_mad_u64_u32 v[16:17], s[16:17], %15, %18, v[16:17]\n\t"
+        "v_mad_u64_u32 v[16:17], s[16:17], v20, s8, v[16:17]\n\t"
+        "v_mad_u64_u32 v[16:17], s[16:17], v21, s7, v[16:17]\n\t"
+        "v_mad_u64_u32 v[16:17], s[16:17], v22, s6, v[16:17]\n\t"
+        "v_mad_u64_u32 v[16:17], s[16:17], v23, s5, v[16:17]\n\t"
+        "v_not_b32 v24, v16\n\t"
+        "v_and_b32 v24, v27, v24\n\t"
+        "v_ashrrev_i64 v[16:17], 29, v[16:17]\n\t"
+        "v_mad_u64_u32 v[16:17], s[16:17], %9, %25, v[16:17]\n\t"
+        "v_mad_u64_u32 v[16:17], s[16:17], %10, %24, v[16:17]\n\t"
+        "v_mad_u64_u32 v[16:17], s[16:17], %11, %23, v[16:17]\n\t"
+        "v_mad_u64_u32 v[16:17], s[16:17], %12, %22, v[16:17]\n\t"
+        "v_mad_u64_u32 v[16:17], s[16:17], %13, %21, v[16:17]\n\t"
+        "v_mad_u64_u32 v[16:17], s[16:17], %14, %20, v[16:17]\n\t"
+        "v_mad_u64_u32 v[16:17], s[16:17], %15, %19, v[16:17]\n\t"
+        "v_mad_u64_u32 v[16:17], s[16:17], %16, %18, v[16:17]\n\t"
+        "v_mad_u64_u32 v[16:17], s[16:17], v21, s8, v[16:17]\n\t"
+        "v_mad_u64_u32 v[16:17], s[16:17], v22, s7, v[16:17]\n\t"
+        "v_mad_u64_u32 v[16:17], s[16:17], v23, s6, v[16:17]\n\t"
+        "v_mad_u64_u32 v[16:17], s[16:17], v24, s5, v[16:17]\n\t"
+        "v_not_b32 v25, v16\n\t"
+        "v_and_b32 v25, v27, v25\n\t"
+        "v_ashrrev_i64 v[16:17], 29, v[16:17]\n\t"
+        "v_mad_u64_u32 v[16:17], s[16:17], %9, %26, v[16:17]\n\t"
+        "v_mad_u64_u32 v[16:17], s[16:17], %10, %25, v[16:17]\n\t"
+        "v_mad_u64_u32 v[16:17], s[16:17], %11, %24, v[16:17]\n\t"
+        "v_mad_u64_u32 v[16:17], s[16:17], %12, %23, v[16:17]\n\t"
+        "v_mad_u64_u32 v[16:17], s[16:17], %13, %22, v[16:17]\n\t"
+        "v_mad_u64_u32 v[16:17], s[16:17], %14, %21, v[16:17]\n\t"
+        "v_mad_u64_u32 v[16:17], s[16:17], %15, %20, v[16:17]\n\t"
+        "v_mad_u64_u32 v[16:17], s[16:17], %16, %19, v[16:17]\n\t"
+        "v_mad_u64_u32 v[16:17], s[16:17], %17, %18, v[16:17]\n\t"
+        "v_mad_u64_u32 v[16:17], s[16:17], v18, s12, v[16:17]\n\t"
+        "v_mad_u64_u32 v[16:17], s[16:17], v22, s8, v[16:17]\n\t"
+        "v_mad_u64_u32 v[16:17], s[16:17], v23, s7, v[16:17]\n\t"
+        "v_mad_u64_u32 v[16:17], s[16:17], v24, s6, v[16:17]\n\t"
+        "v_mad_u64_u32 v[16:17], s[16:17], v25, s5, v[16:17]\n\t"
+        "v_not_b32 v26, v16\n\t"
+        "v_and_b32 v26, v27, v26\n\t"
+        "v_ashrrev_i64 v[16:17], 29, v[16:17]\n\t"
+        "v_lshl_add_u64 v[16:17], v[16:17], 0, 1\n\t"
+        "v_mad_u64_u32 v[16:17], s[16:17], %10, %26, v[16:17]\n\t"
+        "v_mad_u64_u32 v[16:17], s[16:17], %11, %25, v[16:17]\n\t"
+        "v_mad_u64_u32 v[16:17], s[16:17], %12, %24, v[16:17]\n\t"
+        "v_mad_u64_u32 v[16:17], s[16:17], %13, %23, v[16:17]\n\t"
+        "v_mad_u64_u32 v[16:17], s[16:17], %14, %22, v[16:17]\n\t"
+        "v_mad_u64_u32 v[16:17], s[16:17], %15, %21, v[16:17]\n\t"
+        "v_mad_u64_u32 v[16:17], s[16:17], %16, %20, v[16:17]\n\t"
+        "v_mad_u64_u32 v[16:17], s[16:17], %17, %19, v[16:17]\n\t"
+        "v_mad_u64_u32 v[16:17], s[16:17], v19, s12, v[16:17]\n\t"
+        "v_mad_u64_u32 v[16:17], s[16:17], v23, s8, v[16:17]\n\t"
+        "v_mad_u64_u32 v[16:17], s[16:17], v24, s7, v[16:17]\n\t"
+        "v_mad_u64_u32 v[16:17], s[16:17], v25, s6, v[16:17]\n\t"
+        "v_mad_u64_u32 v[16:17], s[16:17], v26, s5, v[16:17]\n\t"
+        "v_and_b32 %0, v27, v16\n\t"
+        "v_lshrrev_b64 v[16:17], 29, v[16:17]\n\t"
+        "v_mad_u64_u32 v[16:17], s[16:17], %11, %26, v[16:17]\n\t"
+        "v_mad_u64_u32 v[16:17], s[16:17], %12, %25, v[16:17]\n\t"
+        "v_mad_u64_u32 v[16:17], s[16:17], %13, %24, v[16:17]\n\t"
+        "v_mad_u64_u32 v[16:17], s[16:17], %14, %23, v[16:17]\n\t"
+        "v_mad_u64_u32 v[16:17], s[16:17], %15, %22, v[16:17]\n\t"
+        "v_mad_u64_u32 v[16:17], s[16:17], %16, %21, v[16:17]\n\t"
+        "v_mad_u64_u32 v[16:17], s[16:17], %17, %20, v[16:17]\n\t"
+        "v_mad_u64_u32 v[16:17], s[16:17], v20, s12, v[16:17]\n\t"
+        "v_mad_u64_u32 v[16:17], s[16:17], v24, s8, v[16:17]\n\t"
+        "v_mad_u64_u32 v[16:17], s[16:17], v25, s7, v[16:17]\n\t"
+        "v_mad_u64_u32 v[16:17], s[16:17], v26, s6, v[16:17]\n\t"
+        "v_and_b32 %1, v27, v16\n\t"
+        "v_lshrrev_b64 v[16:17], 29, v[16:17]\n\t"
+        "v_mad_u64_u32 v[16:17], s[16:17], %12, %26, v[16:17]\n\t"
+        "v_mad_u64_u32 v[16:17], s[16:17], %13, %25, v[16:17]\n\t"
+        "v_mad_u64_u32 v[16:17], s[16:17], %14, %24, v[16:17]\n\t"
+        "v_mad_u64_u32 v[16:17], s[16:17], %15, %23, v[16:17]\n\t"
+        "v_mad_u64_u32 v[16:17], s[16:17], %16, %22, v[16:17]\n\t"
+        "v_mad_u64_u32 v[16:17], s[16:17], %17, %21, v[16:17]\n\t"
+        "v_mad_u64_u32 v[16:17], s[16:17], v21, s12, v[16:17]\n\t"
+        "v_mad_u64_u32 v[16:17], s[16:17], v25, s8, v[16:17]\n\t"
+        "v_mad_u64_u32 v[16:17], s[16:17], v26, s7, v[16:17]\n\t"
+        "v_and_b32 %2, v27, v16\n\t"
+        "v_lshrrev_b64 v[16:17], 29, v[16:17]\n\t"
+        "v_mad_u64_u32 v[16:17], s[16:17], %13, %26, v[16:17]\n\t"
+        "v_mad_u64_u32 v[16:17], s[16:17], %14, %25, v[16:17]\n\t"
+        "v_mad_u64_u32 v[16:17], s[16:17], %15, %24, v[16:17]\n\t"
+        "v_mad_u64_u32 v[16:17], s[16:17], %16, %23, v[16:17]\n\t"
+        "v_mad_u64_u32 v[16:17], s[16:17], %17, %22, v[16:17]\n\t"
+        "v_mad_u64_u32 v[16:17], s[16:17], v22, s12, v[16:17]\n\t"
+        "v_mad_u64_u32 v[16:17], s[16:17], v26, s8, v[16:17]\n\t"
+        "v_and_b32 %3, v27, v16\n\t"
+        "v_lshrrev_b64 v[16:17], 29, v[16:17]\n\t"
+        "v_mad_u64_u32 v[16:17], s[16:17], %14, %26, v[16:17]\n\t"
+        "v_mad_u64_u32 v[16:17], s[16:17], %15, %25, v[16:17]\n\t"
+        "v_mad_u64_u32 v[16:17], s[16:17], %16, %24, v[16:17]\n\t"
+        "v_mad_u64_u32 v[16:17], s[16:17], %17, %23, v[16:17]\n\t"
+        "v_mad_u64_u32 v[16:17], s[16:17], v23, s12, v[16:17]\n\t"
+        "v_and_b32 %4, v27, v16\n\t"
+        "v_lshrrev_b64 v[16:17], 29, v[16:17]\n\t"
+        "v_mad_u64_u32 v[16:17], s[16:17], %15, %26, v[16:17]\n\t"
+        "v_mad_u64_u32 v[16:17], s[16:17], %16, %25, v[16:17]\n\t"
+        "v_mad_u64_u32 v[16:17], s[16:17], %17, %24, v[16:17]\n\t"
+        "v_mad_u64_u32 v[16:17], s[16:17], v24, s12, v[16:17]\n\t"
+        "v_and_b32 %5, v27, v16\n\t"
+        "v_lshrrev_b64 v[16:17], 29, v[16:17]\n\t"
+        "v_mad_u64_u32 v[16:17], s[16:17], %16, %26, v[16:17]\n\t"
+        "v_mad_u64_u32 v[16:17], s[16:17], %17, %25, v[16:17]\n\t"
+        "v_mad_u64_u32 v[16:17], s[16:17], v25, s12, v[16:17]\n\t"
+        "v_and_b32 %6, v27, v16\n\t"
+        "v_lshrrev_b64 v[16:17], 29, v[16:17]\n\t"
+        "v_mad_u64_u32 v[16:17], s[16:17], %17, %26, v[16:17]\n\t"
+        "v_mad_u64_u32 v[16:17], s[16:17], v26, s12, v[16:17]\n\t"
+        "v_and_b32 %7, v27, v16\n\t"
+        "v_lshrrev_b64 v[16:17], 29, v[16:17]\n\t"
+        "v_mov_b32 %8, v16\n\t"
+        : "=&v"(t.l[0]), "=&v"(t.l[1]), "=&v"(t.l[2]), "=&v"(t.l[3]), "=&v"(t.l[4]), "=&v"(t.l[5]), "=&v"(t.l[6]), "=&v"(t.l[7]), "=&v"(t.l[8])
+        : "v"(a.l[0]), "v"(a.l[1]), "v"(a.l[2]), "v"(a.l[3]), "v"(a.l[4]), "v"(a.l[5]), "v"(a.l[6]), "v"(a.l[7]), "v"(a.l[8]), "v"(b.l[0]), "v"(b.l[1]), "v"(b.l[2]), "v"(b.l[3]), "v"(b.l[4]), "v"(b.l[5]), "v"(b.l[6]), "v"(b.l[7]), "v"(b.l[8])
+        : "v16", "v17", "v18", "v19", "v20", "v21", "v22", "v23", "v24", "v25", "v26", "v27", "s4", "s5", "s6", "s7", "s8", "s9", "s10", "s11", "s12", "s13", "s14", "s15", "s16", "s17", "vcc");
+    return t;
+}
+
+template <>
+__device__ __forceinline__ F29<PallasFq> f29_sqr_p1_asm<PallasFq>(const F29<PallasFq>& a) {
+    F29<PallasFq> t, d;
+#pragma unroll
+    for (int i = 0; i < 9; i++) d.l[i] = a.l[i] << 1;
+    asm(
+        "s_mov_b32 s5, 0x02375908\n\t"
+        "s_mov_b32 s6, 0x052a3763\n\t"
+        "s_mov_b32 s7, 0x0d31f813\n\t"
+        "s_mov_b32 s8, 0x00000224\n\t"
+        "s_mov_b32 s12, 0x00400000\n\t"
+        "v_mov_b32 v27, 0x1fffffff\n\t"
+        "v_mad_u64_u32 v[16:17], s[16:17], %9, %9, -1\n\t"
+        "v_not_b32 v18, v16\n\t"
+        "v_and_b32 v18, v27, v18\n\t"
+        "v_ashrrev_i64 v[16:17], 29, v[16:17]\n\t"
+        "v_mad_u64_u32 v[16:17], s[16:17], %9, %19, v[16:17]\n\t"
+        "v_mad_u64_u32 v[16:17], s[16:17], v18, s5, v[16:17]\n\t"
+        "v_not_b32 v19, v16\n\t"
+        "v_and_b32 v19, v27, v19\n\t"
+        "v_ashrrev_i64 v[16:17], 29, v[16:17]\n\t"
+        "v_mad_u64_u32 v[16:17], s[16:17], %9, %20, v[16:17]\n\t"
+        "v_mad_u64_u32 v[16:17], s[16:17], %10, %10, v[16:17]\n\t"
+        "v_mad_u64_u32 v[16:17], s[16:17], v18, s6, v[16:17]\n\t"
+        "v_mad_u64_u32 v[16:17], s[16:17], v19, s5, v[16:17]\n\t"
+        "v_not_b32 v20, v16\n\t"
+        "v_and_b32 v20, v27, v20\n\t"
+        "v_ashrrev_i64 v[16:17], 29, v[16:17]\n\t"
+        "v_mad_u64_u32 v[16:17], s[16:17], %9, %21, v[16:17]\n\t"
+        "v_mad_u64_u32 v[16:17], s[16:17], %10, %20, v[16:17]\n\t"
+        "v_mad_u64_u32 v[16:17], s[16:17], v18, s7, v[16:17]\n\t"
+        "v_mad_u64_u32 v[16:17], s[16:17], v19, s6, v[16:17]\n\t"
+        "v_mad_u64_u32 v[16:17], s[16:17], v20, s5, v[16:17]\n\t"
+        "v_not_b32 v21, v16\n\t"
+        "v_and_b32 v21, v27, v21\n\t"
+        "v_ashrrev_i64 v[16:17], 29, v[16:17]\n\t"
+        "v_mad_u64_u32 v[16:17], s[16:17], %9, %22, v[16:17]\n\t"
+        "v_mad_u64_u32 v[16:17], s[16:17], %10, %21, v[16:17]\n\t"
+        "v_mad_u64_u32 v[16:17], s[16:17], %11, %11, v[16:17]\n\t"
+        "v_mad_u64_u32 v[16:17], s[16:17], v18, s8, v[16:17]\n\t"
+        "v_mad_u64_u32 v[16:17], s[16:17], v19, s7, v[16:17]\n\t"
+        "v_mad_u64_u32 v[16:17], s[16:17], v20, s6, v[16:17]\n\t"
+        "v_mad_u64_u32 v[16:17], s[16:17], v21, s5, v[16:17]\n\t"
+        "v_not_b32 v22, v16\n\t"
+        "v_and_b32 v22, v27, v22\n\t"
+        "v_ashrrev_i64 v[16:17], 29, v[16:17]\n\t"
+        "v_mad_u64_u32 v[16:17], s[16:17], %9, %23, v[16:17]\n\t"
+        "v_mad_u64_u32 v[16:17], s[16:17], %10, %22, v[16:17]\n\t"
+        "v_mad_u64_u32 v[16:17], s[16:17], %11, %21, v[16:17]\n\t"
+        "v_mad_u64_u32 v[16:17], s[16:17], v19, s8, v[16:17]\n\t"
+        "v_mad_u64_u32 v[16:17], s[16:17], v20, s7, v[16:17]\n\t"
+        "v_mad_u64_u32 v[16:17], s[16:17], v21, s6, v[16:17]\n\t"
+        "v_mad_u64_u32 v[16:17], s[16:17], v22, s5, v[16:17]\n\t"
+        "v_not_b32 v23, v16\n\t"
+        "v_and_b32 v23, v27, v23\n\t"
+        "v_ashrrev_i64 v[16:17], 29, v[16:17]\n\t"
+        "v_mad_u64_u32 v[16:17], s[16:17], %9, %24, v[16:17]\n\t"
+        "v_mad_u64_u32 v[16:17], s[16:17], %10, %23, v[16:17]\n\t"
+        "v_mad_u64_u32 v[16:17], s[16:17], %11, %22, v[16:17]\n\t"
+        "v_mad_u64_u32 v[16:17], s[16:17], %12, %12, v[16:17]\n\t"
+        "v_mad_u64_u32 v[16:17], s[16:17], v20, s8, v[16:17]\n\t"
+        "v_mad_u64_u32 v[16:17], s[16:17], v21, s7, v[16:17]\n\t"
+        "v_mad_u64_u32 v[16:17], s[16:17], v22, s6, v[16:17]\n\t"
+        "v_mad_u64_u32 v[16:17], s[16:17], v23, s5, v[16:17]\n\t"
+        "v_not_b32 v24, v16\n\t"
+        "v_and_b32 v24, v27, v24\n\t"
+        "v_ashrrev_i64 v[16:17], 29, v[16:17]\n\t"
+        "v_mad_u64_u32 v[16:17], s[16:17], %9, %25, v[16:17]\n\t"
+        "v_mad_u64_u32 v[16:17], s[16:17], %10, %24, v[16:17]\n\t"
+        "v_mad_u64_u32 v[16:17], s[16:17], %11, %23, v[16:17]\n\t"
+        "v_mad_u64_u32 v[16:17], s[16:17], %12, %22, v[16:17]\n\t"
+        "v_mad_u64_u32 v[16:17], s[16:17], v21, s8, v[16:17]\n\t"
+        "v_mad_u64_u32 v[16:17], s[16:17], v22, s7, v[16:17]\n\t"
+        "v_mad_u64_u32 v[16:17], s[16:17], v23, s6, v[16:17]\n\t"
+        "v_mad_u64_u32 v[16:17], s[16:17], v24, s5, v[16:17]\n\t"
+        "v_not_b32 v25, v16\n\t"
+        "v_and_b32 v25, v27, v25\n\t"
+        "v_ashrrev_i64 v[16:17], 29, v[16:17]\n\t"
+        "v_mad_u64_u32 v[16:17], s[16:17], %9, %26, v[16:17]\n\t"
+        "v_mad_u64_u32 v[16:17], s[16:17], %10, %25, v[16:17]\n\t"
+        "v_mad_u64_u32 v[16:17], s[16:17], %11, %24, v[16:17]\n\t"
+        "v_mad_u64_u32 v[16:17], s[16:17], %12, %23, v[16:17]\n\t"
+        "v_mad_u64_u32 v[16:17], s[16:17], %13, %13, v[16:17]\n\t"
+        "v_mad_u64_u32 v[16:17], s[16:17], v18, s12, v[16:17]\n\t"
+        "v_mad_u64_u32 v[16:17], s[16:17], v22, s8, v[16:17]\n\t"
+        "v_mad_u64_u32 v[16:17], s[16:17], v23, s7, v[16:17]\n\t"
+        "v_mad_u64_u32 v[16:17], s[16:17], v24, s6, v[16:17]\n\t"
+        "v_mad_u64_u32 v[16:17], s[16:17], v25, s5, v[16:17]\n\t"
+        "v_not_b32 v26, v16\n\t"
+        "v_and_b32 v26, v27, v26\n\t"
+        "v_ashrrev_i64 v[16:17], 29, v[16:17]\n\t"
+        "v_lshl_add_u64 v[16:17], v[16:17], 0, 1\n\t"
+        "v_mad_u64_u32 v[16:17], s[16:17], %10, %26, v[16:17]\n\t"
+        "v_mad_u64_u32 v[16:17], s[16:17], %11, %25, v[16:17]\n\t"
+        "v_mad_u64_u32 v[16:17], s[16:17], %12, %24, v[16:17]\n\t"
+        "v_mad_u64_u32 v[16:17], s[16:17], %13, %23, v[16:17]\n\t"
+        "v_mad_u64_u32 v[16:17], s[16:17], v19, s12, v[16:17]\n\t"
+        "v_mad_u64_u32 v[16:17], s[16:17], v23, s8, v[16:17]\n\t"
+        "v_mad_u64_u32 v[16:17], s[16:17], v24, s7, v[16:17]\n\t"
+        "v_mad_u64_u32 v[16:17], s[16:17], v25, s6, v[16:17]\n\t"
+        "v_mad_u64_u32 v[16:17], s[16:17], v26, s5, v[16:17]\n\t"
+        "v_and_b32 %0, v27, v16\n\t"
+        "v_lshrrev_b64 v[16:17], 29, v[16:17]\n\t"
+        "v_mad_u64_u32 v[16:17], s[16:17], %11, %26, v[16:17]\n\t"
+        "v_mad_u64_u32 v[16:17], s[16:17], %12, %25, v[16:17]\n\t"
+        "v_mad_u64_u32 v[16:17], s[16:17], %13, %24, v[16:17]\n\t"
+        "v_mad_u64_u32 v[16:17], s[16:17], %14, %14, v[16:17]\n\t"
+        "v_mad_u64_u32 v[16:17], s[16:17], v20, s12, v[16:17]\n\t"
+        "v_mad_u64_u32 v[16:17], s[16:17], v24, s8, v[16:17]\n\t"
+        "v_mad_u64_u32 v[16:17], s[16:17], v25, s7, v[16:17]\n\t"
+        "v_mad_u64_u32 v[16:17], s[16:17], v26, s6, v[16:17]\n\t"
+        "v_and_b32 %1, v27, v16\n\t"
+        "v_lshrrev_b64 v[16:17], 29, v[16:17]\n\t"
+        "v_mad_u64_u32 v[16:17], s[16:17], %12, %26, v[16:17]\n\t"
+        "v_mad_u64_u32 v[16:17], s[16:17], %13, %25, v[16:17]\n\t"
+        "v_mad_u64_u32 v[16:17], s[16:17], %14, %24, v[16:17]\n\t"
+        "v_mad_u64_u32 v[16:17], s[16:17], v21, s12, v[16:17]\n\t"
+        "v_mad_u64_u32 v[16:17], s[16:17], v25, s8, v[16:17]\n\t"
+        "v_mad_u64_u32 v[16:17], s[16:17], v26, s7, v[16:17]\n\t"
+        "v_and_b32 %2, v27, v16\n\t"
+        "v_lshrrev_b64 v[16:17], 29, v[16:17]\n\t"
+        "v_mad_u64_u32 v[16:17], s[16:17], %13, %26, v[16:17]\n\t"
+        "v_mad_u64_u32 v[16:17], s[16:17], %14, %25, v[16:17]\n\t"
+        "v_mad_u64_u32 v[16:17], s[16:17], %15, %15, v[16:17]\n\t"
+        "v_mad_u64_u32 v[16:17], s[16:17], v22, s12, v[16:17]\n\t"
+        "v_mad_u64_u32 v[16:17], s[16:17], v26, s8, v[16:17]\n\t"
+        "v_and_b32 %3, v27, v16\n\t"
+        "v_lshrrev_b64 v[16:17], 29, v[16:17]\n\t"
+        "v_mad_u64_u32 v[16:17], s[16:17], %14, %26, v[16:17]\n\t"
+        "v_mad_u64_u32 v[16:17], s[16:17], %15, %25, v[16:17]\n\t"
+        "v_mad_u64_u32 v[16:17], s[16:17], v23, s12, v[16:17]\n\t"
+        "v_and_b32 %4, v27, v16\n\t"
+        "v_lshrrev_b64 v[16:17], 29, v[16:17]\n\t"
+        "v_mad_u64_u32 v[16:17], s[16:17], %15, %26, v[16:17]\n\t"
+        "v_mad_u64_u32 v[16:17], s[16:17], %16, %16, v[16:17]\n\t"
+        "v_mad_u64_u32 v[16:17], s[16:17], v24, s12, v[16:17]\n\t"
+        "v_and_b32 %5, v27, v16\n\t"
+        "v_lshrrev_b64 v[16:17], 29, v[16:17]\n\t"
+        "v_mad_u64_u32 v[16:17], s[16:17], %16, %26, v[16:17]\n\t"
+        "v_mad_u64_u32 v[16:17], s[16:17], v25, s12, v[16:17]\n\t"
+        "v_and_b32 %6, v27, v16\n\t"
+        "v_lshrrev_b64 v[16:17], 29, v[16:17]\n\t"
+        "v_mad_u64_u32 v[16:17], s[16:17], %17, %17, v[16:17]\n\t"
+        "v_mad_u64_u32 v[16:17], s[16:17], v26, s12, v[16:17]\n\t"
+        "v_and_b32 %7, v27, v16\n\t"
+        "v_lshrrev_b64 v[16:17], 29, v[16:17]\n\t"
+        "v_mov_b32 %8, v16\n\t"
+        : "=&v"(t.l[0]), "=&v"(t.l[1]), "=&v"(t.l[2]), "=&v"(t.l[3]), "=&v"(t.l[4]), "=&v"(t.l[5]), "=&v"(t.l[6]), "=&v"(t.l[7]), "=&v"(t.l[8])
+        : "v"(a.l[0]), "v"(a.l[1]), "v"(a.l[2]), "v"(a.l[3]), "v"(a.l[4]), "v"(a.l[5]), "v"(a.l[6]), "v"(a.l[7]), "v"(a.l[8]), "v"(d.l[0]), "v"(d.l[1]), "v"(d.l[2]), "v"(d.l[3]), "v"(d.l[4]), "v"(d.l[5]), "v"(d.l[6]), "v"(d.l[7]), "v"(d.l[8])
+        : "v16", "v17", "v18", "v19", "v20", "v21", "v22", "v23", "v24", "v25", "v26", "v27", "s4", "s5", "s6", "s7", "s8", "s9", "s10", "s11", "s12", "s13", "s14", "s15", "s16", "s17", "vcc");
+    return t;
+}
+
+}
+#endif
diff --git a/lurk_beta_amd/csrc/gen_field29_asm.py b/lurk_beta_amd/csrc/gen_field29_asm.py
--- a/lurk_beta_amd/csrc/gen_field29_asm.py
+++ b/lurk_beta_amd/csrc/gen_field29_asm.py
@@ -9,6 +9,7 @@
 BN254FQ_FIELDS = {
     "Bn254Fq": 0x30644E72E131A029B85045B68181585D97816A916871CA8D3C208C16D87CFD47,
 }
+P1_FIELDS = ("PallasFp", "PallasFq")
 W = 29
 MASK = (1 << W) - 1
 ACC_LO, ACC_HI = 16, 17
@@ -26,9 +27,11 @@
     return [(x >> (W * i)) & MASK for i in range(9)]
 
 
-def gen_mul(modulus, square=False):
+def gen_mul(modulus, square=False, p1=False):
     p = limbs29(modulus)
     inv = (-pow(modulus, -1, 1 << W)) % (1 << W)
+    if p1 and (p[0] != 1 or inv != MASK):
+        raise SystemExit(f"--p1: modulus 0x{modulus:x} is not 1 mod 2^{W}")
     L = []
     T = lambda i: f"%{i}"
     A = lambda i: f"%{9 + i}"
@@ -59,9 +62,16 @@
             prods = [(A(i), B(k - i)) for i in range(max(0, k - 8), min(k, 8) + 1)]
         prods += [(M(i), P(k - i)) for i in range(max(0, k - 8), min(k - 1, 8) + 1) if p[k - i] != 0]
         for x, y in prods:
-            src2 = "0" if first else f"v[{ACC_LO}:{ACC_HI}]"
+            src2 = ("-1" if p1 else "0") if first else f"v[{ACC_LO}:{ACC_HI}]"
             L.append(f"v_mad_u64_u32 v[{ACC_LO}:{ACC_HI}], s[{DUMMY}:{DUMMY + 1}], {x}, {y}, {src2}")
             first = False
+        if k <= 8 and p1:
+            L.append(f"v_not_b32 {M(k)}, v{ACC_LO}")
+            L.append(f"v_and_b32 {M(k)}, v{MASK_VGPR}, {M(k)}")
+            L.append(f"v_ashrrev_i64 v[{ACC_LO}:{ACC_HI}], {W}, v[{ACC_LO}:{ACC_HI}]")
+            if k == 8:
+                L.append(f"v_lshl_add_u64 v[{ACC_LO}:{ACC_HI}], v[{ACC_LO}:{ACC_HI}], 0, 1")
+            continue
         if k <= 8:
             if inv == MASK:
                 L.append(f"v_sub_u32 {M(k)}, 0, v{ACC_LO}")
@@ -78,8 +88,9 @@
     return L, p, inv
 
 
-def cxx_sqr(name, modulus):
-    lines, p, inv = gen_mul(modulus, square=True)
+def cxx_sqr(name, modulus, p1=False):
+    lines, p, inv = gen_mul(modulus, square=True, p1=p1)
+    fn = "f29_sqr_p1_asm" if p1 else "f29_sqr_asm"
     nmad = sum(1 for l in lines if l.startswith("v_mad"))
     body = "\n".join(f'        "{l}\\n\\t"' for l in lines)
     outs = ", ".join(f'"=&v"(t.l[{i}])' for i in range(9))
@@ -88,7 +99,7 @@
     sclob = ", ".join(f'"s{r}"' for r in range(P_SGPR_BASE, DUMMY + 2))
     return f"""// {name} squaring: {nmad} v_mad_u64_u32 (cross products once, against the doubled operand)
 template <>
-__device__ __forceinline__ F29<{name}> f29_sqr_asm<{name}>(const F29<{name}>& a) {{
+__device__ __forceinline__ F29<{name}> {fn}<{name}>(const F29<{name}>& a) {{
     F29<{name}> t, d;
 #pragma unroll
     for (int i = 0; i < 9; i++) d.l[i] = a.l[i] << 1;
@@ -102,8 +113,9 @@
 """
 
 
-def cxx(name, modulus):
-    lines, p, inv = gen_mul(modulus)
+def cxx(name, modulus, p1=False):
+    lines, p, inv = gen_mul(modulus, p1=p1)
+    fn = "f29_mul_p1_asm" if p1 else "f29_mul_asm"
     nmad = sum(1 for l in lines if l.startswith("v_mad"))
     nvalu = sum(1 for l in lines if l.startswith("v_"))
     body = "\n".join(f'        "{l}\\n\\t"' for l in lines)
@@ -113,7 +125,7 @@
     sclob = ", ".join(f'"s{r}"' for r in range(P_SGPR_BASE, DUMMY + 2))
     return f"""// {name}: {nmad} v_mad_u64_u32, {nvalu} VALU instructions, no carry folds
 template <>
-__device__ __forceinline__ F29<{name}> f29_mul_asm<{name}>(const F29<{name}>& a, const F29<{name}>& b) {{
+__device__ __forceinline__ F29<{name}> {fn}<{name}>(const F29<{name}>& a, const F29<{name}>& b) {{
     F29<{name}> t;
     asm(
 {body}
@@ -127,20 +139,31 @@
 
 def main():
     bn254fq = sys.argv[1:] == ["--bn254fq"]
+    p1 = sys.argv[1:] == ["--p1"]
     out = [
         "// field29_mul_asm_bn254fq.cuh - GENERATED by gen_field29_asm.py --bn254fq; do not edit." if bn254fq else
+        "// field29_mul_asm_p1.cuh - GENERATED by gen_field29_asm.py --p1; do not edit." if p1 else
         "// field29_mul_asm.cuh - GENERATED by gen_field29_asm.py; do not edit.",
         "#pragma once",
         "#if defined(__HIP_DEVICE_COMPILE__)",
         "namespace lurk {",
     ]
-    if not bn254fq:
+    if p1:
+        out += [
+            "template <class P> __device__ __forceinline__ F29<P> f29_mul_p1_asm(const F29<P>& a, const F29<P>& b);",
+            "template <class P> __device__ __forceinline__ F29<P> f29_sqr_p1_asm(const F29<P>& a);",
+        ]
+    elif not bn254fq:
         out += [
             "template <class P> __device__ __forceinline__ F29<P> f29_mul_asm(const F29<P>& a, const F29<P>& b);",
             "template <class P> __device__ __forceinline__ F29<P> f29_sqr_asm(const F29<P>& a);",
         ]
     out.append("")
-    for name, mod in (BN254FQ_FIELDS if bn254fq else FIELDS).items():
+    if p1:
+        for name in P1_FIELDS:
+            out.append(cxx(name, FIELDS[name], p1=True))
+            out.append(cxx_sqr(name, FIELDS[name], p1=True))
+    for name, mod in ({} if p1 else BN254FQ_FIELDS if bn254fq else FIELDS).items():
         out.append(cxx(name, mod))
         out.append(cxx_sqr(name, mod))
     out += ["}  // namespace lurk", "#endif"]
```
